# benjjneb/dada2

Hardware: AMD Instinct MI355X
Metric: unique reads denoised/sec (dada() wall-clock) (higher is better)
Workload: dtype int32 DP + f64 lambda/p-value

## Files before the change

### dada2_amd/_lib.py

```python
from __future__ import annotations

import ctypes as C
import os

from .opts import COpts

os.environ.setdefault("GPU_MAX_HW_QUEUES", "8")

_HERE = os.path.dirname(os.path.abspath(__file__))
LIB_PATH = os.path.join(_HERE, "libdada2hip.so")
_lib = None


class Dada2HipError(RuntimeError):
    def __init__(self, code, msg):
        super().__init__(msg)
        self.code = code


class CStats(C.Structure):
    _fields_ = [
        ("ncompare", C.c_uint64), ("nskipped", C.c_uint64), ("nshroud", C.c_uint64), ("ngapless", C.c_uint64),
        ("nnw", C.c_uint64), ("nshuffle", C.c_uint64), ("nstored", C.c_uint64),
        ("rounds", C.c_uint32), ("kernel_times_sampled", C.c_uint32),
        ("ms_total", C.c_double), ("ms_upload", C.c_double), ("ms_screen", C.c_double), ("ms_nw", C.c_double),
        ("ms_gapless", C.c_double), ("ms_bookkeep", C.c_double), ("ms_pval", C.c_double), ("ms_final", C.c_double),
        ("nw_kernel_ms", C.c_double), ("nw_kernel_launches", C.c_uint64), ("nw_cells", C.c_uint64),
        ("screen_kernel_ms", C.c_double), ("screen_kernel_launches", C.c_uint64), ("screen_bytes", C.c_uint64),
        ("dev_ms_screen", C.c_double), ("dev_ms_nw", C.c_double), ("dev_ms_shuffle", C.c_double),
        ("dev_ms_pval", C.c_double), ("dev_ms_birth", C.c_double), ("dev_ms_final", C.c_double),
        ("ms_wait_device", C.c_double), ("ms_replay", C.c_double), ("ms_enqueue", C.c_double),
        ("nmoves", C.c_uint64), ("batch_compares", C.c_uint64),
        ("nnw_run", C.c_uint64), ("ngapless_run", C.c_uint64),
        ("lite_chains", C.c_uint64), ("lite_misses", C.c_uint64),
        ("tail_launches", C.c_uint64), ("tail_pauses", C.c_uint64), ("tail_levels", C.c_uint64),
        ("tail_blocks", C.c_uint32), ("tail_fallbacks", C.c_uint32),
        ("dev_ms_tail", C.c_double), ("tail_ms_entry", C.c_double), ("tail_ms_shuffle0", C.c_double),
        ("tail_ms_shuffle_more", C.c_double), ("tail_ms_pupdate", C.c_double), ("tail_ms_barriers", C.c_double),
        ("tail_ms_birth", C.c_double), ("tail_ms_publish", C.c_double), ("tail_ms_release", C.c_double),
        ("pf_compares", C.c_uint64), ("pf_hits", C.c_uint64), ("pf_waits", C.c_uint64), ("pf_exits", C.c_uint64),
        ("pf_centres", C.c_uint64), ("tail_threads", C.c_uint32), ("overlap_on", C.c_uint32),
        ("dev_ms_pf_screen", C.c_double), ("dev_ms_pf_nw", C.c_double),
        ("tail_xcd_barrier", C.c_uint32), ("tail_mirror", C.c_uint32),
        ("ms_setup", C.c_double), ("ms_round0", C.c_double), ("tail_ms_pf_wait", C.c_double), ("tail_ms_pf_plan", C.c_double),
        ("nnw_retry", C.c_uint64), ("nnw_fast", C.c_uint64), ("screen_stage2", C.c_uint64), ("nnw_rounds", C.c_uint64),
    ]

    def as_dict(self):
        return {k: getattr(self, k) for k, _ in self._fields_ if not k.startswith("reserved")}


EXCHANGE_FN = C.CFUNCTYPE(C.c_int, C.c_void_p, C.c_int32, C.c_void_p, C.c_int64, C.c_void_p)


LOG_FN = C.CFUNCTYPE(None, C.c_char_p, C.c_void_p)
ABORT_FN = C.CFUNCTYPE(C.c_int, C.c_void_p)


class CHooks(C.Structure):
    _fields_ = [("log", LOG_FN), ("should_abort", ABORT_FN), ("user", C.c_void_p)]


def make_hooks(log=None, should_abort=None):
    if log is None and should_abort is None:
        return None, None
    keep = {"error": None}

    def _log(msg, _user):
        try:
            if log is not None:
                log(msg.decode(errors="replace"))
        except BaseException as ex:
            keep["error"] = keep["error"] or ex

    def _abort(_user):
        try:
            return 1 if (should_abort is not None and should_abort()) else 0
        except BaseException as ex:
            keep["error"] = keep["error"] or ex
            return 1

    h = CHooks(LOG_FN(_log), ABORT_FN(_abort), None)
    keep["cb"] = (h.log, h.should_abort)
    return h, keep


class CShard(C.Structure):
    _fields_ = [("rank", C.c_int32), ("world", C.c_int32), ("exchange", EXCHANGE_FN), ("user", C.c_void_p)]


EXPORTS = [
    "dada2hip_dada_uniques", "dada2hip_sample_create", "dada2hip_sample_set_priors", "dada2hip_sample_run",
    "dada2hip_sample_free", "dada2hip_sample_run_sharded", "dada2hip_sample_nraw", "dada2hip_sample_maxlen", "dada2hip_result_nclust",
    "dada2hip_result_nraw", "dada2hip_result_maxlen", "dada2hip_result_ncol", "dada2hip_result_nbirth_subs",
    "dada2hip_result_sequence", "dada2hip_result_abundance", "dada2hip_result_n0", "dada2hip_result_n1",
    "dada2hip_result_nunq", "dada2hip_result_clust_pval", "dada2hip_result_birth_from", "dada2hip_result_birth_pval",
    "dada2hip_result_birth_fold", "dada2hip_result_birth_ham", "dada2hip_result_birth_qave", "dada2hip_result_center",
    "dada2hip_result_bs_pos", "dada2hip_result_bs_ref", "dada2hip_result_bs_sub", "dada2hip_result_bs_qual",
    "dada2hip_result_bs_clust", "dada2hip_result_subqual", "dada2hip_result_clusterquals", "dada2hip_result_map",
    "dada2hip_result_pval", "dada2hip_result_stats", "dada2hip_result_free", "dada2hip_nwalign", "dada2hip_nwvec",
    "dada2hip_sample_compare", "dada2hip_launch_ledger", "dada2hip_nw_ring_trips", "dada2hip_sample_final_worklist", "dada2hip_calc_pA", "dada2hip_version", "dada2hip_run_multi", "dada2hip_trim_cache",
    "dada2hip_table_bimera2", "dada2hip_is_bimera", "dada2hip_bimera_pairs", "dada2hip_derep_fastq", "dada2hip_derep_nuniques",
    "dada2hip_derep_nreads", "dada2hip_derep_maxlen", "dada2hip_derep_seqs", "dada2hip_derep_abundances",
    "dada2hip_derep_quals", "dada2hip_derep_map", "dada2hip_derep_free", "dada2hip_sample_from_derep",
    "dada2hip_merge_pairs", "dada2hip_mergers_nrow", "dada2hip_mergers_sequence", "dada2hip_mergers_abundance",
    "dada2hip_mergers_forward", "dada2hip_mergers_reverse", "dada2hip_mergers_nmatch", "dada2hip_mergers_nmismatch",
    "dada2hip_mergers_nindel", "dada2hip_mergers_prefer", "dada2hip_mergers_accept", "dada2hip_mergers_free",
    "dada2hip_collapse_nomismatch", "dada2hip_collapse_pairs", "dada2hip_nweval",
    "dada2hip_taxonomy_train", "dada2hip_taxonomy_free", "dada2hip_taxonomy_table", "dada2hip_taxonomy_assign",
    "dada2hip_species_open", "dada2hip_species_free", "dada2hip_species_match", "dada2hip_species_hits_offsets",
    "dada2hip_species_hits_refs", "dada2hip_species_hits_free",
    "dada2hip_filter_open", "dada2hip_filter_free", "dada2hip_filter_reads", "dada2hip_filter_fastq", "dada2hip_filter_fastq_paired",
    "dada2hip_filter_reads_oriented", "dada2hip_filter_fastq_oriented", "dada2hip_filter_fastq_paired_ex",
    "dada2hip_primers_reads", "dada2hip_primers_fastq",
    "dada2hip_derep_combine", "dada2hip_sample_set_prior_seqs", "dada2hip_sample_prior_seqs_stats",
    "dada2hip_qprofile_reads", "dada2hip_qprofile_fastq", "dada2hip_qprofile_ncycle", "dada2hip_qprofile_counts",
    "dada2hip_qprofile_reads_total", "dada2hip_qprofile_profiled", "dada2hip_qprofile_qual_offset", "dada2hip_qprofile_free",
    "dada2hip_complexity_reads", "dada2hip_complexity_fastq", "dada2hip_complexity_free",
    "dada2hip_bimera_denovo", "dada2hip_bimera_worklist_probe", "dada2hip_bimera_fold_probe",
    "dada2hip_derep_reads", "dada2hip_filter_derep_fastq", "dada2hip_filter_derep_fastq_paired",
    "dada2hip_seqtab_merge", "dada2hip_seqtab_nrow", "dada2hip_seqtab_ncol", "dada2hip_seqtab_cells", "dada2hip_seqtab_sequences",
    "dada2hip_seqtab_samples", "dada2hip_seqtab_free",
    "dada2hip_merge_run", "dada2hip_merge_run_nsamples", "dada2hip_merge_run_nrow", "dada2hip_merge_run_column", "dada2hip_merge_run_sequences",
    "dada2hip_merge_run_free",
]

BIMERA_DENOVO_NSTATS = 16
BIMERA_DENOVO_STATS = ("sequences", "rows", "queries", "pairs_possible", "pairs_aligned", "windows", "launches", "flagged", "aligner_route",
                       "per", "slot_budget", "pack_us", "device_us", "kernel_device_us", "total_us")

PRIOR_SEQS_NSTATS = 16
PRIOR_SEQS_STATS = ("given", "kept", "keys", "keys_in_lds", "flags_set", "blocks", "pack_us", "device_us", "kernel_device_us", "total_us")


class CDerepView(C.Structure):
    _fields_ = [("nuniques", C.c_int32), ("maxlen", C.c_int32), ("nreads", C.c_int64), ("seqs", C.c_void_p),
                ("abundances", C.c_void_p), ("quals", C.c_void_p), ("map", C.c_void_p)]

COLLAPSE_NSTATS = 16
COLLAPSE_STATS = ("columns_dedup", "candidate_pairs", "pairs_scanned", "pairs_screened_out", "pairs_bound_rejected", "pairs_aligned",
                  "aligned_ham0", "batches", "join_us", "scan_us", "align_us", "resolve_us", "total_us")

TAXONOMY_NSTATS = 16
TAXONOMY_TRAIN_STATS = ("build_us", "upload_us", "table_bytes")
TAXONOMY_STATS = ("classified", "slab_queries", "gather_queries", "took_reverse_complement", "launches", "prepare_us", "slab_device_us",
                  "gather_device_us", "try_rc_device_us", "total_us")

SPECIES_NSTATS = 16
SPECIES_STATS = ("references", "bases", "windows", "windows_past_bitmap", "candidates", "candidate_reruns", "hits", "launches",
                 "seed_host_us", "seed_device_us", "verify_host_us", "verify_device_us", "total_us", "resident_bytes")

FILTER_NSTATS = 32
FILTER_STAGES = ("kept", "max_len", "trim_left", "trim_right", "trunc_q", "trunc_len", "min_len", "max_n", "min_q", "max_ee", "rm_phix",
                 "rm_lowcomplex")
FILTER_STATS = ("reads_in", "reads_kept") + tuple("dropped_" + s for s in FILTER_STAGES[1:]) + (
    "table_keys", "table_in_lds", "upload_bytes", "upload_us", "scan_device_us", "ee_device_us", "kmers_device_us", "download_us",
    "parse_us", "deflate_us", "write_us", "total_us", "open_inflate_us")


class CFilterParams(C.Structure):
    _fields_ = [("trunc_q", C.c_int32), ("trunc_len", C.c_int32), ("trim_left", C.c_int32), ("trim_right", C.c_int32),
                ("max_len", C.c_int32), ("min_len", C.c_int32), ("max_n", C.c_int32), ("min_q", C.c_int32),
                ("max_ee", C.c_double), ("rm_lowcomplex", C.c_double),
                ("rm_phix", C.c_int32), ("min_matches", C.c_int32), ("non_overlapping", C.c_int32), ("kmer_size", C.c_int32),
                ("qual_offset", C.c_int32), ("reserved", C.c_int32)]


PRIMERS_NSTATS = 24
PRIMER_CODES = ("kept", "no_fwd", "no_rev", "nothing_left", "bad_letter")
PRIMERS_STATS = ("reads_in", "reads_kept") + tuple("dropped_" + s for s in PRIMER_CODES[1:]) + (
    "flipped", "multiple_matches", "hits_fwd", "hits_rev", "pieces", "tiles", "upload_bytes", "upload_us", "kernel_device_us",
    "download_us", "parse_us", "deflate_us", "write_us", "total_us", "open_inflate_us")


class CPrimerParams(C.Structure):
    _fields_ = [("primer_fwd", C.c_char_p), ("primer_rev", C.c_char_p), ("max_mismatch", C.c_int32), ("trim_fwd", C.c_int32),
                ("trim_rev", C.c_int32), ("orient", C.c_int32), ("allow_indels", C.c_int32), ("reserved", C.c_int32)]


READQC_NSTATS = 16
QPROFILE_NSCORE = 94
READQC_STATS = ("reads_in", "reads_profiled", "pieces", "cycles", "upload_bytes", "upload_us", "kernel_device_us", "download_us", "parse_us",
                "total_us", "open_inflate_us")


SEQTAB_NSTATS = 24
SEQTAB_STATS = ("tables", "input_columns", "distinct_sequences", "flagged_sequences", "output_rows", "output_columns", "table_capacity",
                "rebuilds", "collision_rounds", "rc_failed_compares", "pieces", "upload_bytes", "download_bytes", "upload_us", "identity_us",
                "rc_lookup_us", "accumulate_us", "download_us", "total_us")

MERGE_NSTATS = 16
MERGE_STATS = ("samples", "read_pairs_in", "pairs_na", "unique_pairs", "chunks", "accepted", "table_capacity", "collisions", "upload_bytes",
               "download_bytes", "upload_us", "tally_us", "align_us", "eval_us", "download_us", "total_us")

DEREP_NSTATS = 16
DEREP_STATS = ("reads_in", "uniques", "table_capacity", "rebuilds", "collision_rounds", "pieces", "upload_bytes", "download_bytes", "upload_us",
               "kernel_device_us", "download_us", "finalise_us", "total_us")


class CSampleInput(C.Structure):
    _fields_ = [("nraw", C.c_int32), ("quals_nrow", C.c_int32), ("seqs", C.POINTER(C.c_char_p)),
                ("abundances", C.c_void_p), ("priors", C.c_void_p), ("quals", C.c_void_p)]
# ... 215 lines not shown
```

### dada2_amd/csrc/driver.cpp

```cpp
#include <fcntl.h>
#include <sys/file.h>
#include <unistd.h>

#include <algorithm>
#include <atomic>
#include <chrono>
#include <condition_variable>
#include <exception>
#include <functional>
#include <mutex>
#include <cmath>
#include <cstdarg>
#include <cstdio>
#include <cstring>
#include <ctime>
#include <memory>
#include <thread>
#include <unordered_map>

#include "engine.h"
#include "hostpar.h"
#include "knobs.h"
#include "marshal.h"
#include "ppois.h"
// ... 1240 lines not shown
    const double pA = (have ? p0 : 1.0) * N;
    if (pA < o.omegaA && have) { b.yes = true; b.type = 'A'; b.c = c; b.pval = pA; }
    else {
      BudTie cp;
      double p1 = 1.0;
      const bool havep = pick(1, cp, p1);
      const double pP = havep ? p1 : 1.0;
      if (pP < o.omegaP && havep) { b.yes = true; b.type = 'P'; b.c = cp; b.pval = pP; }
    }
    if (b.yes) b.newi = nclust_dev;
    return b;
  }

  void launch_birth(const Birth &b) {
    const int raw = b.c.raw;
    if (b.newi >= ccap) grow_clusters(std::max(ccap * 2, b.newi + 1));
    const int ev = ev_begin(EV_BIRTH, profile_all);
    launch_apply_bud(P, s->D, d_creads_snap.p, raw, b.newi, b.c.from, s->h_reads[raw], b.c.from_reads - s->h_reads[raw],
                     s->d_ctab.p, ro_next()->cnt, s->stream);
    ev_end(ev);
    nclust_dev = b.newi + 1;
    snap_fresh = true;
    ri ^= 1;
    if (shard) {
      if ((int)h_upd.size() <= b.newi) h_upd.resize(b.newi + 1, 0);
      h_upd[b.newi] = 1; h_upd[b.c.from] = 1;
    }
  }

  void confirm_auto_birth(const Birth &b) {
    if (b.type != 'A' || b.c.raw != h_rout.p->bud.ties[0][0].raw || !spec_launched)
      throw RuntimeErr{DADA2HIP_ERR_RUNTIME, "dada2hip: internal error: device and host bud decisions differ"};
    nclust_dev = b.newi + 1;
    snap_fresh = true;
    ri ^= 1;
    confirm_spec(b.newi, b.c.raw);
  }

  void record_birth(const Birth &b) {
    const int raw = b.c.raw;
    const int from = clust_of[raw];
    if (from != b.c.from) throw RuntimeErr{DADA2HIP_ERR_RUNTIME, "dada2hip: internal error: host/device membership diverged"};
    const double expected = b.c.comp_lam * bi[from].reads;
    Bi &bf = bi[from];
    const int slot = slot_of[raw];
    const uint32_t last = bf.raw.back();
    bf.raw[slot] = last;
    slot_of[last] = slot;
    bf.raw.pop_back();
    bf.reads -= s->h_reads[raw];
    bi.emplace_back();
    const int newi = (int)bi.size() - 1;
    Bi &nb = bi[newi];
    nb.birth_type = b.type;
    nb.birth_from = b.type == 'A' ? (uint32_t)from : 0u;
    nb.birth_pval = b.pval; nb.birth_fold = s->h_reads[raw] / expected; nb.birth_e = expected;
    nb.birth_comp = Comp{(uint32_t)b.c.comp_i, (uint32_t)raw, b.c.comp_lam, b.c.comp_ham};
    nb.raw.push_back((uint32_t)raw);
    nb.reads = s->h_reads[raw];
    nb.center = (uint32_t)raw;
    slot_of[raw] = 0;
    clust_of[raw] = newi;
    if (slot == 0) push_slot0();
    if (b.type == 'A') logf(", Division (naive): Raw %d from Bi %d, pA=%.2e", raw, from, b.pval);
    else logf(", Division (prior): Raw %d, pP=%.2e", raw, b.pval);
  }

  void check_errflag(int32_t f) {
    if (f & 1) throw RuntimeErr{DADA2HIP_ERR_RUNTIME, "Bad lambda."};
    if (f & 2) throw RuntimeErr{DADA2HIP_ERR_RUNTIME, "dada2hip: comparison store overflow"};
    if (f & 32) throw RuntimeErr{DADA2HIP_ERR_RUNTIME, "dada2hip: internal error: a work list of a batch compare overflowed (the compare ran twice?)"};
    if (f & 16) throw RuntimeErr{DADA2HIP_ERR_RUNTIME, "dada2hip: internal error: the persistent tail's LDS mirror disagrees with the state arrays"};
  }

  bool use_v2 = false;
  Eng2 E2{}, E2L{};
  DevBuf<double> v2_lam0, v2_lam1;
  DevBuf<uint32_t> v2_ham0, v2_ham1;
  DevBuf<int32_t> v2_i1;
  DevBuf<unsigned long long> v2_smask;
  DevBuf<int32_t> v2_head, v2_blkcount, v2_dlt, v2_movers, v2_slotc, v2_sig, v2_n0d, v2_blist, v2_blistn;
  DevBuf<unsigned long long> v2_retrytot;
  DevBuf<int32_t> v2_bretry, v2_bretryn;
  DevBuf<double> v2_lamB;
  DevBuf<uint32_t> v2_hamB;
  DevBuf<uint8_t> v2_moved;
  DevBuf<uint32_t> v2_statpart;
  DevBuf<CompBlk> v2_blk;
  DevBuf<Ctl2> v2_ctl;
  DevBuf<BudTie> v2_tiesrec;
  DevBuf<Round2Out> v2_dblk;
  DevBuf<uint16_t> v2_bcls, v2_full, v2_ord;
  DevBuf<uint2> v2_tab8;
  DevBuf<uint32_t> v2_cbits, v3_pf_cbits;
  PinBuf<Round2Out> v2_hblk;
  DevBuf<unsigned long long> v2_trace;
  int v2_trace_seq = -1;
  int v2_nbuf = 64, v2_depth = 2, v2_chain = SH_CHAIN;
  bool v2_debug = false;
  bool v3_on = false;
  int v3_depth = 1;
  int v3_grid = 1;
  long v3_enq = 0;
  long v3_ord_seen = 0;
  DevBuf<PSync> v3_psync;
  DevBuf<int32_t> v3_lockbuf;
  int v3_lock_stride = 0;
  bool v3_overlap = false;
  Eng2 E2P{};
  SampleDev S2{};
  DevBuf<Ctl2> v3_pfctl;
  DevBuf<PfSync> v3_pfsync;
  DevBuf<uint2> v3_pf_tab8;
  DevBuf<uint16_t> v3_pf_full, v3_pf_ord, v3_pf_foff;
  DevBuf<int32_t> v3_pf_blist, v3_pf_blistn, v3_pf_bretry, v3_pf_bretryn;
  DevBuf<uint32_t> v3_pf_ad;
  DevBuf<AdDesc> v3_pf_fdesc;
  long v3_pf_launched = 0;
  long v3_pf_seen = 0;
  long v3_pf_chains = 0;
  bool v3_pf_gate_on = true;
  hipEvent_t v3_pf_ev[4] = {nullptr, nullptr, nullptr, nullptr};
  DevBuf<unsigned long long> v3_ktime;
  PinBuf<int32_t> v3_hflags;
  bool v3_slot_held = false;
  int v3_slot_blocks = 0;
  long v2_enq = 0, v2_cons = 0;
  uint64_t v2_miss_launches = 0;
  struct EnqRec { int ev_screen, ev_nw; bool compare; };
  std::vector<EnqRec> v2_enqrec;

  bool want_v2() const {
    if (knobs().engine_classic) return false;
    if (plain || no_auto || !rounds_use_coop()) return false;
    if (s->D.N < 2) return false;
    return true;
  }
  void v2_bind() {
    E2.P = P; E2.S = s->D;
    E2.T.lam0 = v2_lam0.p; E2.T.ham0 = v2_ham0.p; E2.T.lam1 = v2_lam1.p; E2.T.ham1 = v2_ham1.p; E2.T.i1 = v2_i1.p; E2.T.smask = v2_smask.p; E2.T.head = v2_head.p; E2.T.blk = v2_blk.p; E2.T.blk_count = v2_blkcount.p;
    E2.T.blk_cap = (int32_t)std::min<size_t>(v2_blk.n, 0x7FFFFFF0u);
    E2.C.NBUF = v2_nbuf; E2.C.bcls = v2_bcls.p; E2.C.slot_centre = v2_slotc.p;
    E2.C.tab8 = v2_tab8.p; E2.C.full = v2_full.p; E2.C.ord = v2_ord.p; E2.C.cbits = v2_cbits.p; E2.C.Npad = ((size_t)N + 31) & ~(size_t)15;
    E2.C.lamB = v2_lamB.p; E2.C.hamB = v2_hamB.p; E2.blist = v2_blist.p; E2.blist_n = v2_blistn.p; E2.bretry = v2_bretry.p; E2.bretry_n = v2_bretryn.p; E2.fast_ctl = v2_retrytot.p;
    E2.ctl = v2_ctl.p; E2.dblk = v2_dblk.p; E2.hblk = v2_hblk.p; E2.dlt = v2_dlt.p; E2.movers = v2_movers.p;
    E2.partial = d_partial.p; E2.ties0 = d_ties0.p; E2.ties1 = d_ties1.p; E2.ccap = ccap;
    E2.sig_list = v2_sig.p + 4; E2.sig_n = v2_sig.p; E2.ties_rec = v2_tiesrec.p;
    E2.greedy = o.greedy; E2.detect_singletons = o.detect_singletons;
    E2.total_reads = (double)(uint32_t)s->total_reads; E2.omegaA = o.omegaA; E2.omegaP = o.omegaP;
    E2.bp = BudParams{o.min_fold, o.omegaA, o.omegaP, o.min_hamming, o.min_abund};
    E2.sp = sp; E2.thresh = d_thresh_round.p; E2.max_shuffle = MAX_SHUFFLE;
    E2.trace = v2_trace.p; E2.trace_seq = v2_trace_seq;
    E2.moved = v2_moved.p; E2.n0d = v2_n0d.p; E2.stat_part = v2_statpart.p; E2.stat_n = v2_n0d.p + 2 * SH_LEVELS;
    E2.psync = v3_psync.p; E2.hcons = v3_hflags.p; E2.hexit = v3_hflags.p ? v3_hflags.p + 16 : nullptr; E2.ktime = v3_ktime.p;
    E2.sh_filter = 1; E2.grid_shuffle = 2048; E2.grid_pupdate = 1024;
    const Knobs &K = knobs();
    if (K.v2_filter >= 0) E2.sh_filter = K.v2_filter;
    if (K.v2_grid_shuffle > 0) E2.grid_shuffle = std::min(8192, K.v2_grid_shuffle);
    E2.grid_shuffle = std::max<int>(E2.grid_shuffle, (int)std::min<long long>(8192, (long long)N / (256ll * 1000) + 1));
    if (K.v2_grid_pupdate > 0) E2.grid_pupdate = K.v2_grid_pupdate;
    E2.mov_inline = MOV_INLINE2; E2.ring_limit = RING2;
    if (K.v2_mov_inline > 0) E2.mov_inline = std::min(MOV_INLINE2, K.v2_mov_inline);
    if (K.v3_ring > 0) E2.ring_limit = std::min(RING2, K.v3_ring);
    E2.fail_ordinal = K.v3_fail_entry > 0 ? K.v3_fail_entry : 0;
    E2.grid_wait_ticks = (unsigned long long)((2.0 + (double)N / 1e6) * 1e8);
    E2.spec_lock_buf = v3_lockbuf.p; E2.spec_lock_stride = v3_lock_stride;
    E2.spec_eval = K.v3_spec != 0 ? 1 : 0;
    {
      const long long per_group = 4096ll * std::max(1, v3_grid);
      const long long per_block = ((long long)N + per_group - 1) / per_group * 4096ll;
      E2.mirror_on = (v3_on && K.v3_mirror != 0 && N < (1 << 24) && per_block <= (long long)tail_mirror_cap(s->device)) ? (K.v3_mirror == 2 ? 2 : 1) : 0;
    }
    E2.xbar = K.v3_xbar >= 0 ? K.v3_xbar : (v3_grid >= 48 ? 1 : 0);
    E2.spec_max_prev = K.v3_spec_max >= 0 ? K.v3_spec_max : 16;
    E2.pf_on = v3_overlap ? 1 : 0; E2.pf_min = 2; E2.pf_plan = E2.pf_on;
    E2.pf_early = K.v3_pf_early >= 0 ? K.v3_pf_early : 4;
    E2.pf_sync = K.v3_pf_sync != 0 ? 1 : 0;
    E2.pf_ctl = v3_pfctl.p; E2.pf_blist_n = v3_pf_blistn.p; E2.pfsync = v3_pfsync.p;
    {
      const double us = K.v3_pf_wait_us >= 0 ? (double)K.v3_pf_wait_us : 100.0;
      E2.pf_wait_ticks = (unsigned long long)(us * 100.0);
      v3_pf_gate_on = K.v3_pf_gate_us != 0;
      E2.pf_gate_ticks = (unsigned long long)((K.v3_pf_gate_us > 0 ? (double)K.v3_pf_gate_us : 5000.0) * 100.0);
    }
    E2.has_compare = 1;
    E2.align_at_commit = v2_align_commit ? 1 : 0;
    E2L = E2; E2L.has_compare = 0;
    if (v3_overlap) {
      S2 = s->D; S2.ad_ptr = v3_pf_ad.p; S2.ad_foff = v3_pf_foff.p; S2.ad_desc = v3_pf_fdesc.p;
      E2P = E2; E2P.S = S2; E2P.ctl = v3_pfctl.p; E2P.C.tab8 = v3_pf_tab8.p; E2P.C.full = v3_pf_full.p; E2P.C.ord = v3_pf_ord.p; E2P.C.cbits = v3_pf_cbits.p;
      E2P.blist = v3_pf_blist.p; E2P.blist_n = v3_pf_blistn.p; E2P.bretry = v3_pf_bretry.p; E2P.bretry_n = v3_pf_bretryn.p; E2P.pf_on = 0; E2P.has_compare = 1;
    }
  }
  void v2_alloc(int max_clust) {
    const size_t n = (size_t)N;
    v2_nbuf = 64;
    {
      size_t total_b = 0;
      int dev_ = 0;
      (void)hipGetDevice(&dev_);
      if (hipDeviceTotalMem(&total_b, dev_) != hipSuccess || !total_b) { (void)hipGetLastError(); total_b = (size_t)64 << 30; }
      const size_t per_buf = (((size_t)N + 31) & ~(size_t)15) * (2 + (size_t)KB_MAX * 12);
      v2_nbuf = (int)std::max<size_t>(2, std::min<size_t>(64, total_b / 8 / std::max<size_t>(per_buf, 1)));
    }
    const Knobs &K = knobs();
    if (K.v2_nbuf > 0) v2_nbuf = std::min(64, K.v2_nbuf);
    v2_depth = K.v2_depth > 0 ? std::min(MOV_RING - 1, K.v2_depth) : 2;
    v3_depth = K.v2_depth > 0 ? v2_depth : 1;
    v2_chain = K.v2_chain > 0 ? std::min(SH_CHAIN, K.v2_chain) : SH_CHAIN;
    v2_debug = K.v2_debug;
    hipStream_t stq = s->stream;
    v2_lam0.alloc(n); v2_ham0.alloc(n); v2_lam1.alloc(n); v2_ham1.alloc(n); v2_i1.alloc(n); v2_smask.alloc(n); v2_head.alloc(n); v2_blkcount.alloc(1);
    {
      size_t cap0 = std::max<size_t>(4 * n, (size_t)1 << 16);
      if (K.node_cap > 0) cap0 = std::max<size_t>((size_t)K.node_cap, n + 16);
      if (v2_blk.n < cap0) v2_blk.alloc(cap0);
    }
    v2_ctl.alloc(1); v2_dblk.alloc(RING2); v2_hblk.alloc(RING2);
    v2_dlt.alloc((size_t)SH_LEVELS * ccap);
    v2_movers.alloc((size_t)std::max(MOV_RING * SH_CHAIN, SH_LEVELS) * 3 * n);
    const size_t slots = (size_t)v2_nbuf * KB_MAX;
    v2_bcls.alloc((size_t)v2_nbuf * (((size_t)N + 31) & ~(size_t)15));
    v2_lamB.alloc(slots * (((size_t)N + 31) & ~(size_t)15)); v2_hamB.alloc(slots * (((size_t)N + 31) & ~(size_t)15));
    v2_blist.alloc((size_t)2 * KB_MAX * (((size_t)N + 31) & ~(size_t)15)); v2_blistn.alloc(2 * KB_MAX);
    v2_bretry.alloc((size_t)KB_MAX * (((size_t)N + 31) & ~(size_t)15)); v2_bretryn.alloc(KB_MAX);
    D2_HIP(hipMemsetAsync(v2_blistn.p, 0, 2 * KB_MAX * 4, stq));
    D2_HIP(hipMemsetAsync(v2_bretryn.p, 0, KB_MAX * 4, stq));
    v2_retrytot.alloc(4);
    D2_HIP(hipMemsetAsync(v2_retrytot.p, 0, 32, stq));
    v2_slotc.alloc(slots); v2_tab8.alloc(NKMER); v2_cbits.alloc(KB_MAX * 32); v2_full.alloc((size_t)KB_MAX * NKMER); v2_ord.alloc((size_t)KB_MAX * s->D.LK + 64);
    v2_sig.alloc(n + 4); v2_tiesrec.alloc((size_t)2 * TIES_FULL);
    v2_moved.alloc(n); v2_n0d.alloc(2 * SH_LEVELS + 4); v2_statpart.alloc((size_t)4 * 8192);
    D2_HIP(hipMemsetAsync(v2_moved.p, 0, n, stq));
    D2_HIP(hipMemsetAsync(v2_n0d.p, 0, (2 * SH_LEVELS + 4) * 4, stq));
    D2_HIP(hipMemsetAsync(v2_sig.p, 0, 16, stq));
    D2_HIP(hipMemsetAsync(v2_blkcount.p, 0, 4, stq));
    D2_HIP(hipMemsetAsync(v2_dblk.p, 0, sizeof(Round2Out) * RING2, stq));
    D2_HIP(hipMemsetAsync(v2_dlt.p, 0, (size_t)SH_LEVELS * ccap * 4, stq));
    D2_HIP(hipMemsetAsync(v2_slotc.p, 0xFF, slots * 4, stq));
    for (int k = 0; k < RING2; k++) v2_hblk.p[k].seq = 0;
    Ctl2 c;
    memset(&c, 0, sizeof c);
    c.nclust = 1; c.centre = (int32_t)bi[0].center; c.slot = 0; c.max_clust = max_clust;
    c.n0 = N; c.low0 = N; c.need_compare = 0; c.nalign = 0; c.abuf = 0; c.stable = 1; c.bfrom = 0;
    c.pf_bbuf = -1; c.last_bbuf = -1; c.prev_bbuf = -1;
    for (int k = 0; k < KB_MAX; k++) c.acentre[k] = -1;
    for (int k = 0; k < KB_MAX; k++) c.bcentre[k] = -1;
    D2_HIP(hipMemcpyAsync(v2_ctl.p, &c, sizeof c, hipMemcpyHostToDevice, stq));
    D2_HIP(hipStreamSynchronize(stq));
    v2_trace_seq = -1;
    if (K.v2_trace_on) {
      v2_trace_seq = K.v2_trace_seq;
      v2_trace.alloc((size_t)TRACE_KERNELS * TRACE_BLOCKS * 8);
      D2_HIP(hipMemsetAsync(v2_trace.p, 0, (size_t)TRACE_KERNELS * TRACE_BLOCKS * 64, stq));
    }
    v2_enq = v2_cons = 0;
    v2_next_full = 0;
    v2_lite_on = true;
    if (K.v2_lite >= 0) v2_lite_on = K.v2_lite != 0;
    v2_align_commit = nw_ad_apw(s->D, ap) == 1;
    if (K.v2_align >= 0) v2_align_commit = K.v2_align == 1;
    if (v2_align_commit) v2_lite_on = false;
    v2_plain_rounds = 0;
    v2_miss_launches = 0;
    v2_enqrec.clear();
    v3_setup(stq);
    v2_bind();
  }

  void v3_setup(hipStream_t stq) {
    const Knobs &K = knobs();
    v3_on = !K.v2_tail_chain;
    if (v2_trace_seq >= 0 || K.v2_trace_on) v3_on = false;

    v3_grid = tail_grid(N, s->device);
    if (K.v3_grid > 0) v3_grid = std::min(K.v3_grid, tail_grid(1 << 30, s->device));
    v3_overlap = v3_on && !v2_align_commit && v2_nbuf >= 4 && K.v3_overlap != 0 && N >= 2 && (active_runs(s->device).load() <= 1 || K.v3_overlap == 1);
    {
      const int ncu = tail_grid(1 << 30, s->device);
      if (v3_overlap && K.v3_grid == 0 && v3_grid > ncu / 2) v3_grid = std::max(1, std::min((N + 8191) / 8192, ncu / 2));
    }
    if (v3_on) { const int cap = tail_resident_max(s->device); if (cap == 0 || (cap > 0 && v3_grid > cap)) v3_on = false; }
    if (!v3_on) v3_overlap = false;
    v3_lock_stride = 0;
    if (v3_on) {
      const long long per_group = 4096ll * v3_grid;
      v3_lock_stride = (int)(((long long)N + per_group - 1) / per_group * 4096ll);
      v3_lockbuf.alloc((size_t)v3_lock_stride * (size_t)v3_grid);
    }
    v3_pf_launched = 0; v3_pf_seen = 0; v3_pf_chains = 0;
    if (v3_overlap) {
      if (!s->cmp) D2_HIP(hipStreamCreateWithFlags(&s->cmp, hipStreamNonBlocking));
      for (auto &e : v3_pf_ev) if (!e) D2_HIP(hipEventCreateWithFlags(&e, hipEventDisableTiming));
      const size_t npad = ((size_t)N + 31) & ~(size_t)15;
      v3_pfctl.alloc(1); v3_pfsync.alloc(1); v3_pf_tab8.alloc(NKMER); v3_pf_cbits.alloc(KB_MAX * 32); v3_pf_full.alloc((size_t)KB_MAX * NKMER);
      v3_pf_ord.alloc((size_t)KB_MAX * s->D.LK + 64); v3_pf_blist.alloc((size_t)2 * KB_MAX * npad); v3_pf_blistn.alloc(2 * KB_MAX);
      v3_pf_bretry.alloc((size_t)KB_MAX * npad); v3_pf_bretryn.alloc(KB_MAX);
      D2_HIP(hipMemsetAsync(v3_pf_bretryn.p, 0, KB_MAX * 4, stq));
      v3_pf_ad.alloc((size_t)s->D.ad_waves * s->D.ad_wpw);
      v3_pf_foff.alloc((size_t)s->D.ad_fcap * s->D.ad_fstride); v3_pf_fdesc.alloc((size_t)s->D.ad_fcap);
      D2_HIP(hipMemsetAsync(v3_pf_fdesc.p, 0xFF, (size_t)s->D.ad_fcap * sizeof(AdDesc), stq));
      D2_HIP(hipMemsetAsync(v3_pfctl.p, 0, sizeof(Ctl2), stq));
      D2_HIP(hipMemsetAsync(v3_pfsync.p, 0, sizeof(PfSync), stq));
      D2_HIP(hipMemsetAsync(v3_pf_blistn.p, 0, 2 * KB_MAX * 4, stq));
    }
    v3_psync.alloc(1); v3_hflags.alloc(64); v3_ktime.alloc(KT_N);
    D2_HIP(hipMemsetAsync(v3_psync.p, 0, sizeof(PSync), stq));
    D2_HIP(hipMemsetAsync(v3_ktime.p, 0, KT_N * 8, stq));
    for (int k = 0; k < 64; k++) v3_hflags.p[k] = 0;
    v3_enq = 0; v3_ord_seen = 0;
  }
  bool v3_acquire() {
    if (v3_slot_held) return true;
    v3_slot_blocks = v3_grid;
    persistent_slot(s->device).acquire(std::max(1, knobs().v3_slots), v3_slot_blocks, tail_grid(1 << 30, s->device));
    if (!persistent_file(s->device).try_acquire(s->device)) { persistent_slot(s->device).release(v3_slot_blocks); return false; }
    v3_slot_held = true;
    return true;
  }
  void v3_release() {
    if (v3_slot_held) { persistent_file(s->device).release(); persistent_slot(s->device).release(v3_slot_blocks); v3_slot_held = false; }
  }
  void v3_quiesce() {
    if (!v2_ctl.p || !s) return;
    v3_hflags.p[24] = 1;
    *(volatile int32_t *)(v3_hflags.p + 32) = 1;
    (void)hipMemcpyAsync(&v2_ctl.p->state, v3_hflags.p + 24, 4, hipMemcpyHostToDevice, s->side);
    (void)hipStreamSynchronize(s->side);
    (void)hipStreamSynchronize(s->stream);
    if (s->cmp) (void)hipStreamSynchronize(s->cmp);
    (void)hipGetLastError();
    v3_pf_release();
  }
  void v3_pf_release() {
    v3_pf_ad.free(); v3_pf_foff.free(); v3_pf_fdesc.free(); v3_pf_blist.free(); v3_pf_bretry.free();
  }
  void v3_fallback() {
    sync_spin(s->stream);
    if (v3_overlap) {
      *(volatile int32_t *)(v3_hflags.p + 32) = 1;
      sync_spin(s->cmp);
      v3_pf_totals();
      v3_overlap = false;
      v2_bind();
      v3_pf_release();
    }
    D2_HIP(hipMemsetAsync(v3_psync.p, 0, sizeof(PSync), s->stream));
    launch2_resume(E2, s->stream, true, true);
    v3_release();
    v3_on = false;
    st.tail_fallbacks++;
    v2_enq = v2_cons;
    v2_enqrec.assign((size_t)v2_cons, EnqRec{-1, -1, false});
    v2_next_full = 0;
    if (knobs().v2_summary) fprintf(stderr, "[v3] entry barrier failed after %ld blocks: continuing on the launch chains\n", v2_cons);
  }
  bool v3_block_ready() const { return *(volatile int32_t *)&v2_hblk.p[v2_cons % RING2].seq == (int32_t)(v2_cons + 1); }
  long v3_ended() const { return (long)*(volatile int32_t *)(v3_hflags.p + 16); }
  std::vector<EnqRec> v3_rec;
  void v3_enqueue(bool first) {
    const auto t_enq = clk::now();
    hipStream_t stq = s->stream;
    EnqRec rec{-1, -1, !first};
    if (!first) {
      rec.ev_screen = ev_begin(EV_SCREEN, profile_all, true);
      launch2_screen_multi(E2, stq);
      ev_end(rec.ev_screen);
      launch2_batch_lists(E2, stq);
      const NwBatch nb{&v2_ctl.p->nalign, v2_blistn.p, v2_blist.p, v2_ctl.p->acentre, &v2_ctl.p->abuf, E2.C.Npad, v2_bretry.p, v2_bretryn.p, v2_retrytot.p, &v2_ctl.p->fast_off};
      launch_gapless_batch(s->D, nb, ap, s->d_err.p, v2_lamB.p, v2_hamB.p, &v2_ctl.p->state, stq);
      rec.ev_nw = ev_begin(EV_NW, profile_all, true);
      launch_nw_ad(s->D, -1, nullptr, nullptr, nullptr, 0, nullptr, nullptr, ap, s->d_err.p, v2_lamB.p, v2_hamB.p, nullptr, 0, 0, nullptr, stq,
                   &v2_ctl.p->state, &nb);
      ev_end(rec.ev_nw);
    }
    const int ev = ev_begin(EV_TAIL, profile_all);
    Eng2 Ek = E2;
    if (!profile_all) Ek.ktime = nullptr;
    Ek.pf_plan = (v3_overlap && (active_runs(s->device).load() <= 1 || knobs().v3_overlap == 1)) ? 1 : 0;
    launch3_tail(Ek, v3_grid, first, (int)(v3_enq + 1), s->h_reads[bi[0].center], stq);
    ev_end(ev);
    v3_rec.push_back(rec);
    v3_enq++;
    st.ms_enqueue += ms_since(t_enq);
  }

  void v3_pf_enqueue(long k) {
    const auto t_enq = clk::now();
    hipStream_t st2 = s->cmp;
    Ctl2 *pc = v3_pfctl.p;
    *(volatile int32_t *)(v3_hflags.p + 40 + (k & 7)) = 0;
    launch2_pf_gate(E2P, (int)k, v3_hflags.p + 32, v3_hflags.p + 40 + (k & 7), st2);
    launch2_pf_tables(E2P, st2);
    int ev = ev_begin(EV_PF_SCREEN, profile_all, false, false, st2);
    launch2_screen_multi(E2P, st2);
    ev_end(ev);
    launch2_batch_lists(E2P, st2);
    const NwBatch nb{&pc->nalign, v3_pf_blistn.p, v3_pf_blist.p, pc->acentre, &pc->abuf, E2.C.Npad, v3_pf_bretry.p, v3_pf_bretryn.p, v2_retrytot.p, &pc->fast_off};
    launch_gapless_batch(S2, nb, ap, s->d_err.p, v2_lamB.p, v2_hamB.p, &pc->state, st2);
    ev = ev_begin(EV_PF_NW, profile_all, false, false, st2);
    launch_nw_ad(S2, -1, nullptr, nullptr, nullptr, 0, nullptr, nullptr, ap, s->d_err.p, v2_lamB.p, v2_hamB.p, nullptr, 0, 0, nullptr, st2,
                 &pc->state, &nb);
    ev_end(ev);
    launch2_pf_done(E2P, st2);
    D2_HIP(hipEventRecord(v3_pf_ev[k & 3], st2));
    v3_pf_launched = std::max(v3_pf_launched, k);
    v3_pf_chains++;
    st.ms_enqueue += ms_since(t_enq);
  }
  int v3_pf_gate_result(long k) const { return (int)*(volatile int32_t *)(v3_hflags.p + 40 + (k & 7)); }
  int32_t v3_pf_stat[4] = {0, 0, 0, 0};
  void v3_pf_totals() {
    PfSync ps;
    D2_HIP(hipMemcpy(&ps, v3_pfsync.p, sizeof ps, hipMemcpyDeviceToHost));
    st.nnw_run += ps.nnw; st.ngapless_run += ps.ngapless;
    st.pf_compares = (uint64_t)v3_pf_seen;
    st.pf_hits = (uint64_t)v3_pf_stat[0]; st.pf_waits = (uint64_t)v3_pf_stat[1]; st.pf_exits = (uint64_t)v3_pf_stat[2]; st.pf_centres = (uint64_t)v3_pf_stat[3];
    st.overlap_on = 1;
  }
  void v3_pf_serve(const Round2Out &b) {
    if (!v3_overlap) return;
    for (int k = 0; k < 4; k++) v3_pf_stat[k] = b.pf_stat[k];
    v3_pf_seen = std::max(v3_pf_seen, (long)b.pf_seq);
    if (v3_pf_seen >= 1) {
      if (v3_pf_launched < v3_pf_seen) v3_pf_enqueue(v3_pf_seen);
      else if (v3_pf_gate_result(v3_pf_seen) == 2) v3_pf_enqueue(v3_pf_seen);
    }
    if (v3_pf_gate_on && (active_runs(s->device).load() <= 1 || knobs().v3_overlap == 1) && v3_pf_launched == v3_pf_seen &&
        (v3_pf_seen == 0 || v3_pf_gate_result(v3_pf_seen) == 1))
      v3_pf_enqueue(v3_pf_seen + 1);
    if (b.pf_wait > 0 && (long)b.pf_wait <= v3_pf_launched) D2_HIP(hipStreamWaitEvent(s->stream, v3_pf_ev[b.pf_wait & 3], 0));
  }

  bool v3_dev_halted = false;

  void v3_topup() {
    if (v3_dev_halted) return;
    const long need = (long)v3_depth - (v3_enq - v3_ended());
    for (long k = 0; k < need; k++) v3_enqueue(false);
  }
  const Round2Out &v3_wait_block() {
    const int ring = (int)(v2_cons % RING2);
    const int32_t want = (int32_t)(v2_cons + 1);
    volatile int32_t *seqp = &v2_hblk.p[ring].seq;
    const auto tw = clk::now();
    const bool polite = wait_blocks();
    int burst = 0;
    for (unsigned spins = 0; *seqp != want; spins++) {
      if (v3_enq - v3_ended() < v3_depth && burst < 256) { v3_enqueue(false); burst++; continue; }
      cpu_relax();
      if (polite && spins > 64) { struct timespec ts{0, 20000}; nanosleep(&ts, nullptr); }
      if ((spins & 0xFFFF) == 0xFFFF || (polite && (spins & 0xFF) == 0xFF)) {
        hipError_t e = hipStreamQuery(s->stream);
        if (e != hipSuccess && e != hipErrorNotReady)
          throw d2::DeviceError{DADA2HIP_ERR_DEVICE, std::string("HIP error: ") + hipGetErrorString(e) + " (round result)"};
        if (e == hipSuccess && *seqp != want) {
          if (v3_ended() < v3_enq || burst >= 2) {
            PSync ps;
            D2_HIP(hipMemcpy(&ps, v3_psync.p, sizeof ps, hipMemcpyDeviceToHost));
            if (ps.fail == 1u) throw TailEntryFailed{};
            if (ps.fail != 0u || v3_ended() < v3_enq || burst >= 512)
              throw d2::DeviceError{DADA2HIP_ERR_DEVICE, "dada2hip: the persistent round tail ended without publishing its result (a grid barrier timed out?)"};
          }
          v3_enqueue(false); burst++; continue;
        }
        if (ms_since(tw) > wait_timeout_s() * 1e3)
          throw d2::DeviceError{DADA2HIP_ERR_DEVICE, "dada2hip: timed out waiting for the round result"};
      }
    }
    std::atomic_thread_fence(std::memory_order_acquire);
    v2_cons++;
    st.ms_wait_device += ms_since(tw);
    return v2_hblk.p[ring];
  }

  void run_v3(int max_clust) {
    struct SlotGuard { Run *r; ~SlotGuard() { if (r->v3_running) r->v3_quiesce(); r->v3_release(); r->v3_running = false; } } slot_guard{this};
    v3_running = true;
    auto t0 = clk::now();
    st.nstored = (uint64_t)N;
    v3_rec.clear();
    if (v3_overlap && v3_pf_gate_on && (active_runs(s->device).load() <= 1 || knobs().v3_overlap == 1)) v3_pf_enqueue(1);
    v3_enqueue(true);
    bool done = false;
    long n_halt[8] = {0, 0, 0, 0, 0, 0, 0, 0}, n_pause = 0, n_blocks = 0;
    while (!done) {
      for (int burst = 0; !v3_dev_halted && v3_enq - v3_ended() < v3_depth && burst < 4; burst++) v3_enqueue(false);
      const long seq = v2_cons + 1;
      const Round2Out *bp = nullptr;
      try { bp = &v3_wait_block(); }
      catch (const TailEntryFailed &) {
        v3_running = false;
        v3_fallback();
        st.ms_bookkeep += ms_since(t0);
        run_v2(max_clust, true, v2_cons == 0);
        return;
      }
      const Round2Out &b = *bp;
      n_blocks++;
      v3_pf_serve(b);
      if (hooks && hooks->should_abort && hooks->should_abort(hooks->user))
        throw RuntimeErr{DADA2HIP_ERR_ABORTED, "dada2hip: aborted by caller"};
      if (v2_debug)
        fprintf(stderr, "[v3] blk %ld launch %d halt %d paused %d nclust %d nsh %d cnt %d %d %d %d nbatch %d slot %d birth %d found %d nties %d p %.3e blk %d\n", seq,
                b.kord, b.halt, b.paused, b.nclust, b.nsh, b.cnt[0], b.cnt[1], b.cnt[2], b.cnt[3], b.nbatch, b.slot, b.birth_applied, b.bud.found[0],
                b.bud.nties[0], b.bud.best_p[0], b.blk_count);
      v3_dev_halted = b.halt != H2_NONE;
      v2_replay(b, seq, b.paused != 0 && b.halt == H2_NONE);
      n_halt[b.halt & 7]++;
      if (b.kord > v3_ord_seen) {
        v3_ord_seen = b.kord;
        const EnqRec &rec = v3_rec[(size_t)b.kord - 1];
        if (rec.compare && b.pad0[1] + b.pad0[2] > 0) {
          if (rec.ev_nw >= 0) evs[rec.ev_nw].ok = 1;
          st.nnw_run += (uint64_t)b.pad0[1]; st.ngapless_run += (uint64_t)b.pad0[2];
        }
        if (rec.compare && b.nbatch > 0) {
          v2_miss_launches++;
          if (rec.ev_screen >= 0) evs[rec.ev_screen].ok = 1;
        }
      }
      switch (b.halt) {
        case H2_NONE: {
          Birth bb = decide_bud(b.bud);
          if (!bb.yes || bb.type != 'A' || bb.c.raw != b.bud.ties[0][0].raw)
            throw RuntimeErr{DADA2HIP_ERR_RUNTIME, "dada2hip: internal error: device and host bud decisions differ"};
          logf("\nNew Cluster C%i:", bb.newi);
          nclust_dev = bb.newi + 1;
          record_birth(bb);
          st.ncompare += (uint64_t)N;
          if (b.paused) n_pause++;
          break;
        }
        case H2_NO_BIRTH: {
          Birth bb = decide_bud(b.bud);
          if (bb.yes) throw RuntimeErr{DADA2HIP_ERR_RUNTIME, "dada2hip: internal error: device and host bud decisions differ"};
          done = true;
          break;
        }
        case H2_MAXCLUST: done = true; break;
        case H2_HOST_DECIDE:
        case H2_CAPACITY: {
          if (b.halt == H2_CAPACITY) v2_grow(b);
          Birth bb = decide_bud(b.bud);
          if (!bb.yes) { done = true; break; }
          if (bb.newi + 2 > ccap) v2_grow(b);
          logf("\nNew Cluster C%i:", bb.newi);
          launch2_host_birth(E2, bb.c.raw, bb.c.from, s->stream);
          nclust_dev = bb.newi + 1;
          record_birth(bb);
          st.ncompare += (uint64_t)N;
          break;
        }
        case H2_FAIL: throw d2::DeviceError{DADA2HIP_ERR_DEVICE, "dada2hip: a grid barrier of the persistent round tail timed out (blocks not co-resident?)"};
        default: throw RuntimeErr{DADA2HIP_ERR_RUNTIME, "dada2hip: internal error: unexpected halt code from the persistent round tail"};
      }
      v3_dev_halted = false;
      *(volatile int32_t *)v3_hflags.p = (int32_t)v2_cons;
    }
    v3_running = false;
    sync_spin(s->stream);
    if (v3_overlap) {
      *(volatile int32_t *)(v3_hflags.p + 32) = 1;
      sync_spin(s->cmp);
      v3_pf_totals();
      v3_pf_release();
    }
    if (profile_all && v3_ktime.p) {
      unsigned long long kt[KT_N];
      D2_HIP(hipMemcpy(kt, v3_ktime.p, sizeof kt, hipMemcpyDeviceToHost));
      const double ms = 1e3 / 1e8;
      st.tail_ms_shuffle0 = kt[KT_S0] * ms; st.tail_ms_shuffle_more = kt[KT_SL] * ms; st.tail_ms_pupdate = kt[KT_P] * ms;
      st.tail_ms_barriers = (kt[KT_S0_BAR] + kt[KT_SL_BAR] + kt[KT_P_BAR]) * ms; st.tail_ms_birth = kt[KT_BIRTH] * ms;
      st.tail_ms_publish = kt[KT_PUBLISH] * ms; st.tail_ms_entry = kt[KT_LAUNCH] * ms;
      st.tail_levels = kt[KT_LEVELS]; st.tail_ms_release = kt[KT_RELEASE] * ms;
      st.tail_ms_pf_wait = kt[KT_PFWAIT] * ms; st.tail_ms_pf_plan = kt[KT_PLAN] * ms;
      if (knobs().v2_summary) {
        fprintf(stderr, "[v3] block-0 sub-phase ms (kid: 1 commit+shuffle0, 2 later shuffles, 5 p-update, 6 serial end):");
        for (int kid : {1, 2, 5, 6}) { fprintf(stderr, "  kid%d:", kid); for (int ph = 1; ph < 8; ph++) fprintf(stderr, " %.2f", kt[KT_SUB + 8 * kid + ph] * ms); }
        fprintf(stderr, "\n");
      }
    }
    st.tail_xcd_barrier = (E2.xbar && v3_grid > 1) ? 1u : 0u;
    st.tail_mirror = (v3_enq > 0 && E2.mirror_on) ? 1u : 0u;
    st.tail_launches = (uint64_t)v3_enq; st.tail_pauses = (uint64_t)n_pause; st.tail_blocks = (uint32_t)v3_grid; st.tail_threads = 1024;
    if (knobs().v2_summary && v3_overlap)
      fprintf(stderr, "[v3] overlap: prefetch compares %ld in %ld chains (centres %d)  rounds served from a prefetched batch %d  waits inside the launch %d  launches left for one %d\n",
              v3_pf_seen, v3_pf_chains, v3_pf_stat[3], v3_pf_stat[0], v3_pf_stat[1], v3_pf_stat[2]);
    if (knobs().v2_summary)
      fprintf(stderr, "[v3] blocks %ld  launches %ld  grid %d  halts none/nobirth/host/more/cap/max %ld %ld %ld %ld %ld %ld  pauses %ld  ms: wait %.1f replay %.1f enqueue %.1f total %.1f  moves %llu misses %llu\n",
              n_blocks, v3_enq, v3_grid, n_halt[0], n_halt[1], n_halt[2], n_halt[3], n_halt[4], n_halt[5], n_pause, st.ms_wait_device, st.ms_replay,
              st.ms_enqueue, ms_since(t0), (unsigned long long)st.nmoves, (unsigned long long)v2_miss_launches);
    st.ms_bookkeep += ms_since(t0);
  }

  int v2_plain_rounds = 0;
  long v2_next_full = 0;
  bool v2_lite_on = true;
  bool v2_align_commit = false;
  void v2_enqueue_chain(int nlev, bool with_compare, bool store) {
    const auto t_enq = clk::now();
    EnqRec rec{-1, -1, with_compare};
    const bool lite = with_compare && v2_lite_on && v2_plain_rounds >= 1 && v2_enq + 1 < v2_next_full;
    v2_round_launches(nlev, with_compare, store, &rec, lite);
    if (with_compare) v2_plain_rounds++;
    if (lite) st.lite_chains++;
    v2_enqrec.push_back(rec);
    v2_enq++;
    st.ms_enqueue += ms_since(t_enq);
  }
  void v2_round_launches(int nlev, bool with_compare, bool store, EnqRec *recp, bool lite = false) {
    hipStream_t stq = s->stream;
    EnqRec rec{-1, -1, with_compare};
    const Eng2 &E2 = lite ? this->E2L : this->E2;
    if (with_compare && !lite) {
      rec.ev_screen = ev_begin(EV_SCREEN, profile_all, true);
      launch2_screen_multi(E2, stq);
      ev_end(rec.ev_screen);
      launch2_batch_lists(E2, stq);
      const NwBatch nb{&v2_ctl.p->nalign, v2_blistn.p, v2_blist.p, v2_ctl.p->acentre, &v2_ctl.p->abuf, E2.C.Npad, v2_bretry.p, v2_bretryn.p, v2_retrytot.p, &v2_ctl.p->fast_off};
      launch_gapless_batch(s->D, nb, ap, s->d_err.p, v2_lamB.p, v2_hamB.p, &v2_ctl.p->state, stq);
      rec.ev_nw = ev_begin(EV_NW, profile_all, true);
      launch_nw_ad(s->D, -1, nullptr, nullptr, nullptr, 0, nullptr, nullptr, ap, s->d_err.p, v2_lamB.p, v2_hamB.p, nullptr, 0, 0, nullptr, stq,
                   &v2_ctl.p->state, &nb);
      ev_end(rec.ev_nw);
    }
    int ev = ev_begin(EV_SHUFFLE, profile_all && nlev > 0);
    for (int l = 0; l < nlev; l++) launch2_shuffle(E2, l, store && l == 0, stq);
    ev_end(ev);
    ev = ev_begin(EV_PVAL, profile_all);
    launch2_eval(E2, nlev, s->h_reads[bi[0].center], stq);
    ev_end(ev);
    if (recp) *recp = rec;
  }

  const Round2Out &v2_wait_block() {
    const int ring = (int)(v2_cons % RING2);
    const int32_t want = (int32_t)(v2_cons + 1);
    volatile int32_t *seqp = &v2_hblk.p[ring].seq;
    const auto tw = clk::now();
    const bool polite = wait_blocks();
    for (unsigned spins = 0; *seqp != want; spins++) {
      cpu_relax();
      if (polite && spins > 64) { struct timespec ts{0, 20000}; nanosleep(&ts, nullptr); }
      if ((spins & 0xFFFF) == 0xFFFF || (polite && (spins & 0xFF) == 0xFF)) {
        hipError_t e = hipStreamQuery(s->stream);
        if (e != hipSuccess && e != hipErrorNotReady)
          throw d2::DeviceError{DADA2HIP_ERR_DEVICE, std::string("HIP error: ") + hipGetErrorString(e) + " (round result)"};
        if (e == hipSuccess && *seqp != want)
          throw d2::DeviceError{DADA2HIP_ERR_DEVICE, "dada2hip: the device did not publish the round result"};
        if (ms_since(tw) > wait_timeout_s() * 1e3)
          throw d2::DeviceError{DADA2HIP_ERR_DEVICE, "dada2hip: timed out waiting for the round result"};
      }
    }
    std::atomic_thread_fence(std::memory_order_acquire);
    v2_cons++;
    st.ms_wait_device += ms_since(tw);
    return v2_hblk.p[ring];
  }

  void v2_replay(const Round2Out &b, long seq, bool resume_after_fetch = false) {
    const auto t_rep = clk::now();
    int tot = 0;
    for (int l = 0; l < b.nsh; l++) tot += b.cnt[l];
    st.nmoves += (uint64_t)tot;
    if (tot <= E2.mov_inline) {
      int off = 0;
      for (int l = 0; l < b.nsh; l++) { replay_moves(b.mov + 3 * off, b.cnt[l]); off += b.cnt[l]; }
    } else {
      const int ring = (int)((seq - 1) % MOV_RING);
      h_big.alloc((size_t)3 * tot);
      size_t off = 0;
      for (int l = 0; l < b.nsh; l++) {
        const int nm = b.cnt[l];
        if (!nm) continue;
        const size_t slot = b.kord ? (size_t)l : (size_t)(ring * SH_CHAIN + l);
        D2_HIP(hipMemcpyAsync(h_big.p + 3 * off, v2_movers.p + slot * 3 * N, (size_t)3 * nm * 4, hipMemcpyDeviceToHost, s->side));
        off += (size_t)nm;
      }
      D2_HIP(hipStreamSynchronize(s->side));
      if (resume_after_fetch) {
        launch2_resume(E2, s->stream, true);
        v3_enqueue(false);
      }
      off = 0;
      for (int l = 0; l < b.nsh; l++) { replay_moves(h_big.p + 3 * off, b.cnt[l]); off += (size_t)b.cnt[l]; }
    }
    st.nshuffle += (uint64_t)b.nsh;
    st.nnw += b.stat[0]; st.ngapless += b.stat[1]; st.nshroud += b.stat[2]; st.nskipped += b.stat[3];
    st.nnw_rounds += b.stat[0] - (uint64_t)b.pad0[3];
    st.nstored += (uint64_t)b.pad0[0];
    st.ms_replay += ms_since(t_rep);
    if (b.err_flag & 4) throw RuntimeErr{DADA2HIP_ERR_RUNTIME, "N-W Align out of range."};
    if (b.err_flag & 8) throw RuntimeErr{DADA2HIP_ERR_RUNTIME, "dada2hip: internal error: a cached compare lacks a comparison its round needs"};
    check_errflag(b.err_flag);
  }

  void v2_grow(const Round2Out &b) {
    sync_spin(s->stream);
    if (nclust_dev + 2 > ccap) {
      grow_clusters(std::max(ccap * 2, nclust_dev + 2));
      v2_dlt.alloc((size_t)SH_LEVELS * ccap);
      D2_HIP(hipMemsetAsync(v2_dlt.p, 0, (size_t)SH_LEVELS * ccap * 4, s->stream));
    }
    if ((size_t)b.blk_count + (size_t)N > v2_blk.n) {
      const size_t cap = std::max(v2_blk.n * 2, (size_t)b.blk_count + 2 * (size_t)N);
      DevBuf<CompBlk> nb;
      nb.alloc(cap);
      D2_HIP(hipMemcpyAsync(nb.p, v2_blk.p, (size_t)b.blk_count * sizeof(CompBlk), hipMemcpyDeviceToDevice, s->stream));
      D2_HIP(hipStreamSynchronize(s->stream));
      std::swap(v2_blk.p, nb.p); std::swap(v2_blk.n, nb.n);
    }
    v2_bind();
  }

  void run_v2(int max_clust, bool resume = false, bool first = true) {
    auto t0 = clk::now();
    if (!resume) st.nstored = (uint64_t)N;
    if (first) v2_enqueue_chain(0, false, false);
    bool done = false;
    double t_decide = 0, t_halt = 0, t_top = 0;
    long n_halt[8] = {0, 0, 0, 0, 0, 0, 0, 0}, n_big = 0, n_kind[5] = {0, 0, 0, 0, 0};
    while (!done) {
      const auto t_loop = clk::now();
      while (v2_enq - v2_cons < v2_depth) v2_enqueue_chain(v2_chain, true, true);
      t_top += ms_since(t_loop);
      const long seq = v2_cons + 1;
      const Round2Out &b = v2_wait_block();
      if (hooks && hooks->should_abort && hooks->should_abort(hooks->user))
        throw RuntimeErr{DADA2HIP_ERR_ABORTED, "dada2hip: aborted by caller"};
      if (b.halt == H2_NONE) while (v2_enq - v2_cons < v2_depth) v2_enqueue_chain(v2_chain, true, true);
      if (v2_debug)
        fprintf(stderr, "[v2] blk %ld halt %d nclust %d nlev %d nsh %d cnt %d %d %d %d nbatch %d slot %d birth %d found %d nties %d p %.3e blk %d\n", seq,
                b.halt, b.nclust, b.nlev, b.nsh, b.cnt[0], b.cnt[1], b.cnt[2], b.cnt[3], b.nbatch, b.slot, b.birth_applied, b.bud.found[0],
                b.bud.nties[0], b.bud.best_p[0], b.blk_count);
      if (b.halt == H2_HOST_DECIDE && knobs().v2_summary) {
        const int nt = b.bud.nties[0];
        bool zero = b.bud.found[0] && nt > 1 && nt <= BUD_TIES, in0 = false, pristine = true;
        int cmin = INT32_MAX, ncmin = 0;
        for (int k = 0; zero && k < nt; k++) {
          const BudTie &t = b.bud.ties[0][k];
          if (t.p != 0.0) zero = false;
          if (clust_of[t.raw] == 0) { in0 = true; if (slot_of[t.raw] != t.raw) pristine = false; }
          if (clust_of[t.raw] < cmin) { cmin = clust_of[t.raw]; ncmin = 1; } else if (clust_of[t.raw] == cmin) ncmin++;
        }
        n_kind[!zero ? 0 : (in0 ? (pristine ? 1 : 2) : (ncmin == 1 ? 3 : 4))]++;
      }
      v2_replay(b, seq);
      n_halt[b.halt & 7]++;
      if (b.cnt[0] + b.cnt[1] + b.cnt[2] + b.cnt[3] > MOV_INLINE2) n_big++;
      const auto t_dec = clk::now();
      const EnqRec &rec = v2_enqrec[seq - 1];
      if (rec.compare && b.pad0[1] + b.pad0[2] > 0) {
        if (rec.ev_nw >= 0) evs[rec.ev_nw].ok = 1;
        st.nnw_run += (uint64_t)b.pad0[1]; st.ngapless_run += (uint64_t)b.pad0[2];
      }
      if (rec.compare && b.nbatch > 0) {
        v2_miss_launches++;
        if (rec.ev_screen >= 0) evs[rec.ev_screen].ok = 1;
        v2_next_full = seq + b.nbatch;
      }
      if (b.nlev > 0 && b.halt != H2_SHUFFLE_MORE) { }
      switch (b.halt) {
        case H2_NONE: {
          Birth bb = decide_bud(b.bud);
          if (!bb.yes || bb.type != 'A' || bb.c.raw != b.bud.ties[0][0].raw)
            throw RuntimeErr{DADA2HIP_ERR_RUNTIME, "dada2hip: internal error: device and host bud decisions differ"};
          logf("\nNew Cluster C%i:", bb.newi);
          nclust_dev = bb.newi + 1;
          record_birth(bb);
          st.ncompare += (uint64_t)N;
          break;
        }
        case H2_NO_BIRTH: {
          Birth bb = decide_bud(b.bud);
          if (bb.yes) throw RuntimeErr{DADA2HIP_ERR_RUNTIME, "dada2hip: internal error: device and host bud decisions differ"};
          done = true;
          break;
        }
        case H2_MAXCLUST: done = true; break;
        case H2_HOST_DECIDE:
        case H2_CAPACITY: {
          v2_enq = v2_cons;
          v2_enqrec.resize((size_t)v2_cons);
          if (b.halt == H2_CAPACITY) v2_grow(b);
          Birth bb = decide_bud(b.bud);
          if (!bb.yes) { done = true; break; }
          if (bb.newi + 2 > ccap) v2_grow(b);
          logf("\nNew Cluster C%i:", bb.newi);
          launch2_host_birth(E2, bb.c.raw, bb.c.from, s->stream);
          v2_next_full = 0;
          nclust_dev = bb.newi + 1;
          record_birth(bb);
          st.ncompare += (uint64_t)N;
          break;
        }
        case H2_NEED_COMPARE: {
          v2_enq = v2_cons;
          v2_enqrec.resize((size_t)v2_cons);
          v2_next_full = 0;
          st.lite_misses++;
          launch2_resume(E2, s->stream, true);
          break;
        }
        case H2_SHUFFLE_MORE: {
          v2_enq = v2_cons;
          v2_enqrec.resize((size_t)v2_cons);
          launch2_resume(E2, s->stream);
          v2_enqueue_chain(v2_chain, false, false);
          break;
        }
        default: throw RuntimeErr{DADA2HIP_ERR_RUNTIME, "dada2hip: internal error: unknown halt code"};
      }
      if (b.halt == H2_NONE) t_decide += ms_since(t_dec); else t_halt += ms_since(t_dec);
    }
    if (knobs().v2_summary)
      fprintf(stderr, "[v2] blocks %ld  halts none/nobirth/host/more/cap/max/need-compare %ld %ld %ld %ld %ld %ld %ld  chains without compare %llu  big-mover blocks %ld  ms: wait %.1f replay %.1f "
                      "enqueue %.1f decide %.1f halt-handling %.1f top-up %.1f total %.1f  moves %llu misses %llu  host decisions other/zero-ties in partition 0 at "
                      "their first slots/... moved/elsewhere, one in the lowest partition/... several %ld %ld %ld %ld %ld\n", v2_cons, n_halt[0], n_halt[1],
              n_halt[2], n_halt[3], n_halt[4], n_halt[5], n_halt[6], (unsigned long long)st.lite_chains, n_big, st.ms_wait_device, st.ms_replay, st.ms_enqueue, t_decide, t_halt, t_top,
              ms_since(t0), (unsigned long long)st.nmoves, (unsigned long long)v2_miss_launches, n_kind[0], n_kind[1], n_kind[2], n_kind[3], n_kind[4]);
    sync_spin(s->stream);
    if (v2_trace_seq >= 0 && v2_trace.p) {
      std::vector<unsigned long long> h((size_t)TRACE_KERNELS * TRACE_BLOCKS * 8);
      D2_HIP(hipMemcpy(h.data(), v2_trace.p, h.size() * 8, hipMemcpyDeviceToHost));
      if (FILE *f = fopen(knobs().v2_trace_file.c_str(), "wb")) { fwrite(h.data(), 8, h.size(), f); fclose(f); }
    }
    st.ms_bookkeep += ms_since(t0);
  }

  uint64_t nw_cells_per_alignment() const {
    const int L = s->D.maxlen;
    if (o.band_size < 0) return (uint64_t)(L + 1) * (L + 1);
    return (uint64_t)(2 * L + 1) * (uint64_t)(o.band_size + 1);
  }
};
// ... 1229 lines not shown
```

### dada2_amd/csrc/engine.h

```cpp
#pragma once
#include <cstddef>
#include <cstdint>
#include <string>
#include <vector>

#include <hip/hip_runtime.h>

#include "../../include/dada2hip.h"
#include "merge_plain.h"

namespace d2 {

constexpr int KMER_SIZE = 5;
constexpr int NKMER = 1024;
constexpr int RANK_SAT = 63;
constexpr int MAX_SHUFFLE = 10;
constexpr int SEQLEN = 9999;
constexpr double TAIL_APPROX_CUTOFF = 1e-7;

enum : uint8_t { CLS_SKIP = 0, CLS_SHROUD = 1, CLS_GAPLESS = 2, CLS_NW = 3 };

struct DeviceError {
  int code;
  std::string msg;
// ... 88 lines not shown
                           int32_t *d_size, int32_t *d_off, int32_t *d_work, int nwork, int32_t *d_chunk_centre, hipStream_t st);
void launch_store(const PartState &P, const SampleDev &S, int ci, int centre, double total_reads, const double *d_lam,
                  const uint32_t *d_ham, const int32_t *d_round_counters, const uint8_t *d_cls, int32_t *d_zero2, hipStream_t st);
struct StoreRound {
  int ci, centre;
  double total_reads;
  const double *lam;
  const uint32_t *ham;
  const int32_t *round_counters;
  const uint8_t *cls;
};
void launch_shuffle(const PartState &P, const SampleDev &S, const uint32_t *d_creads_snap, int32_t *d_movers,
                    int32_t *d_nmovers, int32_t *d_inline, const StoreRound *store, int check_only, int nclust, hipStream_t st);
constexpr int BUD_TIES = 64;
constexpr int TIES_FULL = 4096;
struct BudTie { int32_t raw, comp_i; uint32_t comp_ham; int32_t from; uint32_t from_reads, pad; double comp_lam; double p; };
constexpr double BUD_NEAR = 1e-9;
struct BudOut {
  double best_p[2];
  uint32_t best_reads[2];
  int32_t found[2], nties[2];
  int32_t err_flag, node_count;
  int32_t valid;
  int32_t auto_applied;
  BudTie ties[2][BUD_TIES];
};
constexpr int MOVERS_INLINE = 512;
struct RoundOut {
  int32_t cnt[2];
  int32_t seq;
  int32_t pad;
  BudOut bud;
  int32_t mov[2][3 * MOVERS_INLINE];
  int32_t pad_tail[2];
};
void launch_pupdate_bud(const PartState &P, const SampleDev &S, int greedy, int detect_singletons, const BudParams &bp,
                        double init_p, uint32_t init_reads, void *d_partial, BudOut *d_out, int32_t *d_over0, int32_t *d_over1,
                        int nclust, uint8_t *d_lock_tmp, int32_t *d_check_cnt, hipStream_t st);
void launch_apply_bud(const PartState &P, const SampleDev &S, uint32_t *d_creads_snap, int raw, int newi, int from,
                      uint32_t reads_new, uint32_t reads_from, uint32_t *d_ctab, int32_t *d_zero2, hipStream_t st);
void launch_auto_birth(const PartState &P, const SampleDev &S, uint32_t *d_creads_snap, RoundOut *d_block, double omegaA, int newi,
                       uint32_t *d_ctab, int32_t *d_zero2, int32_t *d_next, RoundOut *h_block, int seq, hipStream_t st);
void launch_centre_table(const SampleDev &S, int centre, uint32_t *d_ctab, hipStream_t st);
void launch_final_p(const PartState &P, const SampleDev &S, double omegaC, uint8_t *d_correct, hipStream_t st);
void launch_posthoc(const PartState &P, const SampleDev &S, const int32_t *d_cluster_of_centre, int32_t *d_out_ji, double *d_out_lam,
                    int32_t *d_nout, int cap, hipStream_t st);

void launch_build_kmers(const SampleDev &S, hipStream_t st);
void launch_build_kmers_rows(const SampleDev &S, int r0, int r1, hipStream_t st);
void launch_screen(const SampleDev &S, int centre, const ScreenParams &sp, const uint8_t *d_skip, const uint8_t *d_lock,
                   int greedy, const int32_t *d_thresh, uint8_t *d_cls, double *d_lambda, uint32_t *d_ham, int32_t *d_nw_list,
                   int32_t *d_gl_list, int32_t *d_counters, uint32_t *d_ctab, bool build_table, const int32_t *d_centre_dev,
                   hipStream_t st);
void launch_gapless(const SampleDev &S, int centre, const int32_t *d_chunk_centre, const int32_t *d_work,
                    const int32_t *d_nwork, int nwork_host, const AlignParams &ap, const double *d_err,
                    double *d_lambda, uint32_t *d_ham, uint16_t *d_view, int LV, int view_by_chunk, hipStream_t st);

enum {
  LEDGER_AD = 0,
  LEDGER_AD_LR = 32,
  LEDGER_ADW = 64,
  LEDGER_NW = 72,
  LEDGER_NW_GEN = 88,
  LEDGER_GAPLESS = 96,
  LEDGER_WORDS = 2
};
void ledger_note(int bit);
void ledger_read(uint64_t *out, bool clear);
void nw_trips_note(int trips);
int nw_trips_read(bool clear);
void launch_pair_class(const SampleDev &S, const int32_t *d_pc, const int32_t *d_pr, int n, const ScreenParams &sp,
                       uint8_t *d_out, hipStream_t st);

struct NwScratch {
  uint32_t *ptr = nullptr;
  uint32_t *tcode = nullptr;
  int32_t *rows = nullptr;
  size_t ptr_words_per_wave = 0, t_words_per_wave = 0, row_words_per_wave = 0;
  int nwaves = 0;
};
int nw_class(int band, int maxlen, int minlen);
size_t nw_ptr_words_per_wave(int wclass, int band, int maxlen, int minlen);
void launch_nw(const SampleDev &S, int wclass, int centre, const int32_t *d_chunk_centre, const int32_t *d_work,
               const int32_t *d_nwork, int nwork_host, const AlignParams &ap, const double *d_err, const NwScratch &scr,
               double *d_lambda, uint32_t *d_ham, uint16_t *d_view, int LV, int view_by_chunk, uint8_t *d_moves,
               int moves_stride, int32_t *d_nmoves, hipStream_t st, const int32_t *d_pair_centre = nullptr);

struct NwBatch {
  const int32_t *on;
  const int32_t *n;
  const int32_t *list;
  const int32_t *centre;
  const int32_t *bbuf;
  size_t stride;
  int32_t *retry_list = nullptr;
  int32_t *retry_n = nullptr;
  unsigned long long *fast_ctl = nullptr;
  const int32_t *fast_off = nullptr;
};
void launch_gapless_batch(const SampleDev &S, const NwBatch &b, const AlignParams &ap, const double *d_err, double *d_lambda,
                          uint32_t *d_ham, const int32_t *d_stop_dev, hipStream_t st);
void launch_nw_ad(const SampleDev &S, int centre, const int32_t *d_chunk_centre, const int32_t *d_work,
                  const int32_t *d_nwork, int nwork_host, const int32_t *d_gl_work, const int32_t *d_gl_nwork,
                  const AlignParams &ap, const double *d_err, double *d_lambda, uint32_t *d_ham, uint16_t *d_view, int LV,
                  int view_by_chunk, const int32_t *d_centre_dev, hipStream_t st, const int32_t *d_stop_dev = nullptr,
                  const NwBatch *batch = nullptr);
int nw_ad_apw(const SampleDev &S, const AlignParams &ap);
size_t nw_ad_lds_bytes(const SampleDev &S, const AlignParams &ap);
void launch_nw_ad_lr(const SampleDev &S, const int32_t *d_chunk_centre, const int32_t *d_work, int nwork, const AlignParams &ap,
                     const double *d_err, int allow_one_off, int max_shift, int32_t *d_out, hipStream_t st);
size_t nw_ad_lr_lds_bytes(const SampleDev &S, const AlignParams &ap);

bool nw_adw_ok(const SampleDev &S, const AlignParams &ap);
size_t nw_adw_ptr_words_per_wave(const SampleDev &S, const AlignParams &ap);
int nw_adw_waves(const SampleDev &S, const AlignParams &ap, int nwork);
size_t nw_adw_lds_bytes(const SampleDev &S, const AlignParams &ap);
void launch_nw_adw(const SampleDev &S, int centre, const int32_t *d_chunk_centre, const int32_t *d_work, const int32_t *d_nwork,
                   int nwork_host, const AlignParams &ap, const double *d_err, uint32_t *d_ptr_scr, size_t ptr_wpw,
                   int scr_waves, double *d_lambda, uint32_t *d_ham, uint16_t *d_view, int LV, int view_by_chunk,
                   hipStream_t st);
int nw_adw_apw(const SampleDev &S, const AlignParams &ap);

constexpr int KB_MAX = 8;
constexpr int SH_CHAIN = 4;
constexpr int SH_LEVELS = MAX_SHUFFLE;
#ifndef D2_RING2
#define D2_RING2 16
#endif
constexpr int RING2 = D2_RING2;
constexpr int MOV_RING = 4;
constexpr int TRACE_BLOCKS = 4096, TRACE_KERNELS = 8;
constexpr int MOV_INLINE2 = 32768;

struct alignas(64) CompBlk {
  int32_t next, cnt;
  int32_t i[3];
  uint32_t ham[3];
  double lam[3];
  int32_t pad[2];
};
static_assert(sizeof(CompBlk) == 64, "CompBlk is one 64-byte line");
struct Store2 {
  double *lam0 = nullptr, *lam1 = nullptr;
  uint32_t *ham0 = nullptr, *ham1 = nullptr;
  int32_t *i1 = nullptr;
  unsigned long long *smask = nullptr;
  int32_t *head = nullptr;
  CompBlk *blk = nullptr;
  int32_t *blk_count = nullptr;
  int32_t blk_cap = 0;
};

enum : int32_t { H2_NONE = 0, H2_NO_BIRTH, H2_HOST_DECIDE, H2_SHUFFLE_MORE, H2_CAPACITY, H2_MAXCLUST, H2_NEED_COMPARE, H2_FAIL };

struct Ctl2 {
  int32_t state;
  int32_t halt;
  int32_t nclust;
  int32_t centre;
  int32_t slot;
  int32_t nbatch;
  int32_t bbuf;
  int32_t next_bbuf;
  int32_t pub_seq;
  int32_t nsh_base;
  int32_t max_clust;
  int32_t nalign_ran;
  int32_t nalign, abuf;
  int32_t acentre[KB_MAX];
  int32_t need_compare;
  int32_t n0, low0;
  int32_t bcentre[KB_MAX];
  uint32_t breads[KB_MAX];
  int32_t blen[KB_MAX];
  int32_t kexit, hcons_seen;
  int32_t stable, bfrom;
  int32_t pf_seq, pf_bbuf, last_bbuf, pf_wait;
  int32_t prev_bbuf;
  int32_t pf_hits, pf_spins, pf_exits, pf_centres;
  unsigned long long pf_mask;
  int32_t fast_off, fast_off_pad;
};

struct Cache2 {
  int32_t NBUF = 0;
  uint16_t *bcls = nullptr;
  int32_t *slot_centre = nullptr;
  uint2 *tab8 = nullptr;
  uint16_t *full = nullptr;
  uint16_t *ord = nullptr;
  uint32_t *cbits = nullptr;
  double *lamB = nullptr;
  uint32_t *hamB = nullptr;
  size_t Npad = 0;
};

struct Round2Out {
  int32_t seq;
  int32_t halt;
  int32_t nclust;
  int32_t birth_applied;
  int32_t nlev;
  int32_t nsh;
  int32_t cnt[SH_LEVELS];
  int32_t nbatch;
  int32_t slot;
  int32_t err_flag, blk_count;
  int32_t pad0[4];
  int32_t pf_seq;
  int32_t pf_wait;
  int32_t pf_stat[4];
  int32_t pad1[2];
  int32_t kord;
  int32_t paused;
  unsigned long long stat[4];
  BudOut bud;
  int32_t mov[3 * MOV_INLINE2];
};
static_assert(sizeof(Round2Out) % 16 == 0, "Round2Out is published as uint4s");

struct Eng2 {
  PartState P;
  SampleDev S;
  Store2 T;
  Cache2 C;
  Ctl2 *ctl;
  Round2Out *dblk;
  Round2Out *hblk;
  int32_t *dlt;
  uint8_t *moved;
  int32_t *n0d;
  int32_t *movers;
  uint32_t *stat_part;
  int32_t *stat_n;
  int32_t *blist, *blist_n;
  int32_t *bretry, *bretry_n;
  unsigned long long *fast_ctl;
  void *partial;
  int32_t *ties0, *ties1;
  BudTie *ties_rec;
  int32_t *sig_list, *sig_n;
  int32_t ccap;
  int32_t greedy, detect_singletons;
  double total_reads, omegaA, omegaP;
  BudParams bp;
  ScreenParams sp;
  const int32_t *thresh;
  int32_t max_shuffle;
  unsigned long long *trace;
  int32_t trace_seq;
  int32_t has_compare;
  int32_t align_at_commit;
  int32_t sh_filter;
  int32_t grid_shuffle, grid_pupdate;
  int32_t mov_inline;
  int32_t ring_limit;
  struct PSync *psync;
  volatile int32_t *hcons;
  volatile int32_t *hexit;
  unsigned long long *ktime;
  int32_t xbar;
  int32_t spec_max_prev;
  int32_t spec_eval;
  int32_t fail_ordinal;
  unsigned long long grid_wait_ticks;
  int32_t *spec_lock_buf;
  int32_t spec_lock_stride;
  int32_t mirror_on;
  int32_t pf_on;
  int32_t pf_plan;
  int32_t pf_min;
  int32_t pf_sync;
  int32_t pf_early;
  Ctl2 *pf_ctl;
  int32_t *pf_blist_n;
  struct PfSync *pfsync;
  unsigned long long pf_wait_ticks;
  unsigned long long pf_gate_ticks;
};

struct PfSync {
  uint32_t done, pad0[31];
  unsigned long long nnw, ngapless;
};

struct PSync {
  uint32_t arrive, pad0[31];
  uint32_t gen, pad1[31];
  uint32_t fail, pad2[31];
  uint32_t top, pad3[31];
  uint32_t ngrp, pad4[31];
  uint32_t xarr[8][32], xgen[8][32], xcount[8][32], xn[8][32];
};
enum { KT_S0 = 0, KT_S0_BAR, KT_SL, KT_SL_BAR, KT_P, KT_P_BAR, KT_BIRTH, KT_PUBLISH, KT_ROUNDS, KT_LEVELS, KT_LAUNCH, KT_RELEASE,
       KT_PFWAIT , KT_PLAN , KT_SUB_LAST = 14, KT_SUB = 16, KT_N = 80 };

void launch2_store0(const Eng2 &E, const double *d_lam, const uint32_t *d_ham, const uint8_t *d_cls, const int32_t *d_round_counters,
                    hipStream_t st);
void launch2_screen_multi(const Eng2 &E, hipStream_t st);
void launch2_pf_gate(const Eng2 &E, int k, const int32_t *h_quit, int32_t *h_result, hipStream_t st);
void launch2_pf_tables(const Eng2 &E, hipStream_t st);
void launch2_pf_done(const Eng2 &E, hipStream_t st);
void launch2_batch_lists(const Eng2 &E, hipStream_t st);
void launch2_shuffle(const Eng2 &E, int level, bool store, hipStream_t st);
void launch2_eval(const Eng2 &E, int nlev, uint32_t init_reads, hipStream_t st);
void launch2_host_birth(const Eng2 &E, int raw, int from, hipStream_t st);
void launch2_resume(const Eng2 &E, hipStream_t st, bool keep_list = false, bool compare_done = false);
void launch2_posthoc(const Eng2 &E, const int32_t *d_cluster_of_centre, int32_t *d_out_ji, double *d_out_lam, int32_t *d_nout,
                     int cap, hipStream_t st);
int tail_grid(int N, int device);
int tail_resident_max(int device);
int tail_mirror_cap(int device);
void launch3_tail(const Eng2 &E, int grid, bool first, int ordinal, uint32_t init_reads, hipStream_t st);

void launch_bimera_lr(const SampleDev &S, const int32_t *d_chunk_centre, const int32_t *d_work, int nwork, const uint8_t *d_moves,
                      int stride, const int32_t *d_nmoves, int allow_one_off, int max_shift, int32_t *d_out, hipStream_t st);

void launch_collapse_join(const SampleDev &S, int row0, int nrows, const unsigned long long *d_keys, const int32_t *d_groups,
                          int ngroups, int KW, uint32_t *d_bits, hipStream_t st);
void launch_collapse_scan(const SampleDev &S, const int2 *d_pairs, int npairs, int min_overlap, int match, int mismatch, int use_bound,
                          int4 *d_out, hipStream_t st);
constexpr int TAX_THREADS = 256;
struct TaxPart { float maxlogp; int32_t ntie; uint32_t hash; int32_t genus; };
struct TaxJob {
  const float *T;
  int gpad, ngenus, ntiles, nq, npass;
  const int32_t *koff;
  const uint16_t *karr;
  const long long *boff;
  const uint16_t *bpos;
  const int32_t *qid;
  uint32_t seed_lo, seed_hi;
  TaxPart *part;
  float *best;
  int32_t *ntie, *winner;
};
bool launch_tax_sums(const TaxJob &J, int slab_positions, hipStream_t st);
void launch_tax_combine(const TaxJob &J, hipStream_t st);
constexpr int SP_BITMAP_LOG2 = 18, SP_BITMAP_WORDS = 1 << (SP_BITMAP_LOG2 - 5);
struct SpCand { int32_t ref, pos, key; };
struct SpeciesRefs {
  const uint32_t *words, *nplane;
  const long long *woff;
  const int32_t *len;
};
struct SpeciesKeys {
  const unsigned long long *keys;
  const int32_t *groups;
  int ngroups, nkeys;
  const int32_t *key_pat_off, *key_pats, *pat_woff, *pat_len, *pat_query;
  const uint32_t *pat_words;
};
void launch_species_bitmap(const SpeciesKeys &K, uint32_t *d_bitmap, hipStream_t st);
void launch_species_seed(const SpeciesRefs &R, int r0, int r1, const SpeciesKeys &K, const uint32_t *d_bitmap, SpCand *d_cand,
                         unsigned long long cap, unsigned long long *d_counters, hipStream_t st);
void launch_species_verify(const SpeciesRefs &R, const SpeciesKeys &K, const SpCand *d_cand, unsigned long long ncand,
                           unsigned long long *d_hits, unsigned long long hit_cap, unsigned long long *d_counters, hipStream_t st);
constexpr int FT_THREADS = 1024;
constexpr int FT_LDS_MAX = 144 * 1024;
struct FilterTable {
  const unsigned long long *keys;
  const uint8_t *flags;
  int nkeys, word_size;
};
struct FilterArgs {
  int max_len, skip, trim_right, cut_char, trunc_end, min_len, max_n, minq_on, minq_char, ee_on, rm_phix, min_matches, non_overlapping;
  double max_ee;
};
struct FilterOut { int32_t code, off, len, nother, minq, hits_f, hits_r, pad; double ee; };
void launch_filter_scan(const FilterTable &T, const FilterArgs &A, int n, const uint8_t *d_seq, const uint8_t *d_qual,
                        const long long *d_off, FilterOut *d_out, hipStream_t st);
void launch_filter_ee(const FilterArgs &A, int n, const uint8_t *d_qual, const long long *d_off, const double *d_ee_tab,
                      FilterOut *d_out, hipStream_t st);
void launch_filter_kmers(int n, int k, const uint8_t *d_seq, const long long *d_off, const FilterOut *d_out, int32_t *d_counts,
                         hipStream_t st);
constexpr int FT_ORIENT_MAX = 256;
constexpr int FT_CODE_ORIENT = 12;
struct FilterBarcode {
  uint8_t fwd[FT_ORIENT_MAX], comp[FT_ORIENT_MAX];
  int len;
};
void launch_filter_orient(const FilterBarcode &B, int forward_only, int n, const uint8_t *d_seq, const long long *d_off,
                          FilterOut *d_out, hipStream_t st);
void launch_filter_scan_oriented(const FilterTable &T, const FilterArgs &A, int n, const uint8_t *d_seq, const uint8_t *d_qual,
                                 const long long *d_off, FilterOut *d_out, hipStream_t st);
void launch_filter_ee_oriented(const FilterArgs &A, int n, const uint8_t *d_qual, const long long *d_off, const double *d_ee_tab,
                               FilterOut *d_out, hipStream_t st);
void launch_filter_kmers_oriented(int n, int k, const uint8_t *d_seq, const long long *d_off, const FilterOut *d_out, int32_t *d_counts,
                                  hipStream_t st);
constexpr int PR_THREADS = 128;
constexpr int PR_MAXL = 128;
constexpr int PR_MAXMM = 15;
constexpr int PR_TILE_MAX = 64;
constexpr int PR_GRID = 4096;
constexpr int32_t PR_NA = INT32_MIN;
struct PrimerArgs {
  uint8_t sel[4][PR_MAXL];
  int32_t len[4];
  int32_t act[4], nact;
  int32_t mm, nbits, has_rev, orient, trim_fwd, trim_rev, tile;
};
struct PrimerOut { int32_t code, flip, first, last, hits[4]; };
void launch_primers(const PrimerArgs &A, int n, const uint8_t *d_seq, const long long *d_off, PrimerOut *d_out, int32_t *d_starts,
                    hipStream_t st);
constexpr int QP_NSCORE = 94;
constexpr int QP_TILE = 64;
constexpr int QP_THREADS = 1024;
constexpr int QP_ROW = QP_NSCORE + 1;
constexpr int QP_SLICE = 512;
constexpr int QP_GRID_X = 1024;
void launch_qprofile(int n, int ncyc_pad, const uint8_t *d_qual, const long long *d_off, unsigned long long *d_tab, int32_t *d_bad,
                     hipStream_t st);
constexpr int CW_WINDOW_MAX = 1024;
constexpr int CW_GRID = 16384;
struct ComplexityOut { double lo, last; };
void launch_complexity_win(int n, int k, int window, int by, const uint8_t *d_seq, const long long *d_off, const double *d_ylogy,
                           ComplexityOut *d_out, hipStream_t st);
struct PriorKeys {
  const unsigned long long *keys;
  const int32_t *groups;
  int ngroups, nkeys;
  const int32_t *key_row_off, *row_woff, *row_len, *row_seq;
  const uint32_t *row_words;
};
constexpr int PRIOR_LDS_KEYS_MAX = 6144;
int launch_prior_match(const SampleDev &S, const PriorKeys &K, bool lds, int grid_cap, const uint8_t *d_or_flags, int32_t *d_first_match,
                       hipStream_t st);
struct BimeraFold {
  const int32_t *live;
  int nq, r0, wr;
  const int32_t *work;
  const int32_t *rec;
  const int32_t *len, *P;
  int allow_one_off, min_one_off_par_dist;
  int32_t *maxima;
  uint8_t *flags;
  unsigned long long *aligned;
  int last;
  int32_t *next_live, *n_next;
};
void launch_bimera_worklist(const int32_t *d_live, int nq, int r0, int wr, int per, const int32_t *d_rank, const int32_t *d_P,
                            const uint8_t *d_flags, int32_t *d_chunk_centre, int32_t *d_work, hipStream_t st);
void launch_bimera_fold(const BimeraFold &F, hipStream_t st);
void launch_calc_pA(int n, const int32_t *d_reads, const double *d_E, const uint8_t *d_prior, double *d_out,
                    hipStream_t st);
constexpr int DD_EMPTY = -1;
constexpr int DD_PENDING = -2, DD_SKIP = -1;
struct DdRead { long long start, idx; int32_t len, pad; };
struct DdCounters { unsigned long long arena_used; int32_t nuniq, pending, err, minq; };
struct DdState {
  int32_t *tab;
  int cap;
  unsigned long long hmask;
  unsigned long long *u_hash, *u_count, *u_first, *sums;
  long long *u_off;
// ... 44 lines not shown
```

### dada2_amd/csrc/knobs.h

```cpp
#pragma once
#include <algorithm>
#include <atomic>
#include <cstdlib>
#include <cstring>
#include <memory>
#include <mutex>
#include <string>

namespace d2 {

enum { NWK_AUTO = 0, NWK_LANE = 1, NWK_COOP = 2, NWK_WIDE = 3 };

struct Knobs {
  bool engine_classic = false;
  int nw_kernel = 0;
  bool ad_homo = true;
  bool no_speculation = false;
  bool no_autobirth = false;
  int v2_nbuf = 0;
  int v2_depth = 0;
  int v2_chain = 0;
  int v2_lite = -1;
  int v2_align = -1;
  int v2_filter = -1;
  int v2_grid_shuffle = 0;
  int v2_grid_pupdate = 0;
  int v2_mov_inline = 0;
  bool v2_tail_chain = false;
  int v3_grid = 0;
  int v3_ring = 0;
  int v3_overlap = -1;
  int v3_pf_wait_us = -1;
  int v3_pf_early = -1;
  int v3_pf_gate_us = -1;
  int v3_xbar = -1;
  int v3_spec = 1;
  int v3_spec_max = -1;
  int v3_pf_sync = 0;
  int replay_radix_min = 4096;
  int v3_slots = 3;
  int v3_mirror = 1;
  int v3_fail_entry = 0;
  bool v2_debug = false;
  bool v2_summary = false;
  bool v2_trace_on = false;
  int v2_trace_seq = -1;
  std::string v2_trace_file;
  bool profile = false;
  long long node_cap = 0;
  bool wait_block = false;
  double wait_timeout_s = 600.0;
  long long ad_fcap = 0;
  int screen_bits = 1;
  int ad_fast = 1;
  long long nw_ring = 0;
  long long upload_chunk_rows = 0;
  int ad_debug = 0;
  bool bimera_times = false;
  long long bimera_slots = 0;
  int collapse_batch = 0;
  int collapse_scan = 1;
  int collapse_join = 1;
  int tax_slab = 256;
  long long tax_chunk = 0;
  long long filter_piece = 0;
  long long filter_piece_bytes = 0;
  long long primers_piece = 0;
  long long primers_piece_bytes = 0;
  long long primers_tile = 0;
  long long readqc_piece = 0;
  long long readqc_piece_bytes = 0;
  long long derep_piece = 0;
  long long derep_piece_bytes = 0;
  long long derep_table = 0;
  int derep_hash_bits = 64;
  int merge_hash_bits = 64;
  long long merge_chunk = 0;
  int species_cand = 1 << 20;
  int species_chunk = 8192;
  int priors_lds_keys = 4096;
  int priors_grid = 0;
  bool derep_zlib = false;
  bool derep_times = false;
  int host_threads = 0;
  int alloc_cache = -1;
  long long alloc_cache_gb = -1;
  std::string env_text;

  static Knobs from_env() {
    Knobs k;
    auto S = [&k](const char *n) -> const char * {
      const char *e = std::getenv(n);
      if (e) k.env_text.append(n).append(1, '=').append(e).append(1, '\n');
      return e;
    };
    auto I = [&](const char *n, int dflt) -> int { const char *e = S(n); return e ? std::atoi(e) : dflt; };
    auto B = [&](const char *n) -> bool { const char *e = S(n); return e && std::atoi(e) != 0; };
    auto T = [&](const char *n) -> int { const char *e = S(n); return e ? (std::atoi(e) != 0 ? 1 : 0) : -1; };
    if (const char *e = S("DADA2HIP_ENGINE")) k.engine_classic = !std::strcmp(e, "classic");
    if (const char *e = S("DADA2HIP_NW_KERNEL")) k.nw_kernel = !std::strcmp(e, "lane") ? 1 : (!std::strcmp(e, "coop") ? 2 : (!std::strcmp(e, "wide") ? 3 : 0));
    if (const char *e = S("DADA2HIP_AD_HOMO")) k.ad_homo = std::strcmp(e, "0") != 0;
    k.no_speculation = S("DADA2HIP_NO_SPECULATION") != nullptr;
    k.no_autobirth = S("DADA2HIP_NO_AUTOBIRTH") != nullptr;
    k.v2_nbuf = I("DADA2HIP_V2_NBUF", 0); k.v2_depth = I("DADA2HIP_V2_DEPTH", 0); k.v2_chain = I("DADA2HIP_V2_CHAIN", 0);
    k.v2_lite = T("DADA2HIP_V2_LITE");
    if (const char *e = S("DADA2HIP_V2_ALIGN")) k.v2_align = !std::strcmp(e, "commit") ? 1 : 0;
    k.v2_filter = T("DADA2HIP_V2_FILTER");
    k.v2_grid_shuffle = I("DADA2HIP_V2_GRID_SHUFFLE", 0); k.v2_grid_pupdate = I("DADA2HIP_V2_GRID_PUPDATE", 0);
    k.v2_mov_inline = I("DADA2HIP_V2_MOV_INLINE", 0);
    if (const char *e = S("DADA2HIP_V2_TAIL")) k.v2_tail_chain = !std::strcmp(e, "chain");
    k.v3_grid = I("DADA2HIP_V3_GRID", 0); k.v3_ring = I("DADA2HIP_V3_RING", 0);
    k.v3_overlap = T("DADA2HIP_V3_OVERLAP"); k.v3_pf_wait_us = I("DADA2HIP_V3_PF_WAIT_US", -1);
    k.v3_fail_entry = I("DADA2HIP_V3_FAIL_ENTRY", 0); k.v3_spec = I("DADA2HIP_V3_SPEC", 1); k.v3_xbar = T("DADA2HIP_V3_XBAR"); k.v3_spec_max = I("DADA2HIP_V3_SPEC_MAX", -1);
    k.v3_pf_early = I("DADA2HIP_V3_PF_EARLY", -1); k.v3_pf_sync = I("DADA2HIP_V3_PF_SYNC", 0); k.v3_pf_gate_us = I("DADA2HIP_V3_PF_GATE_US", -1);
    k.v3_mirror = I("DADA2HIP_V3_MIRROR", 1);
    k.v3_slots = I("DADA2HIP_V3_SLOTS", 3);
    k.replay_radix_min = I("DADA2HIP_REPLAY_RADIX_MIN", 4096);
    k.v2_debug = S("DADA2HIP_V2_DEBUG") != nullptr; k.v2_summary = S("DADA2HIP_V2_SUMMARY") != nullptr;
    if (const char *e = S("DADA2HIP_V2_TRACE")) {
      k.v2_trace_on = true; k.v2_trace_seq = std::atoi(e);
      const char *colon = std::strchr(e, ':');
      k.v2_trace_file = colon ? colon + 1 : "dada2hip_trace.bin";
    }
    k.profile = B("DADA2HIP_PROFILE");
    if (const char *e = S("DADA2HIP_NODE_CAP")) k.node_cap = std::atoll(e);
    if (const char *e = S("DADA2HIP_WAIT")) k.wait_block = !std::strcmp(e, "block");
    if (const char *e = S("DADA2HIP_WAIT_TIMEOUT_S")) k.wait_timeout_s = std::atof(e);
    if (const char *e = S("DADA2HIP_AD_FCAP")) k.ad_fcap = std::atoll(e);
    k.ad_debug = I("DADA2HIP_AD_DEBUG", 0); k.ad_fast = I("DADA2HIP_AD_FAST", 1); k.screen_bits = I("DADA2HIP_SCREEN_BITS", 1);
    if (const char *e = S("DADA2HIP_BIMERA_TIMES")) k.bimera_times = !std::strcmp(e, "1");
    k.collapse_batch = I("DADA2HIP_COLLAPSE_BATCH", 0); k.collapse_scan = I("DADA2HIP_COLLAPSE_SCAN", 1);
    k.collapse_join = I("DADA2HIP_COLLAPSE_JOIN", 1);
    k.tax_slab = I("DADA2HIP_TAX_SLAB", 256);
    auto P = [&](const char *n) -> long long { const char *e = S(n); return e ? std::max(1ll, std::atoll(e)) : 0ll; };
    k.tax_chunk = P("DADA2HIP_TAX_CHUNK"); k.filter_piece = P("DADA2HIP_FILTER_PIECE"); k.filter_piece_bytes = P("DADA2HIP_FILTER_PIECE_BYTES");
    k.upload_chunk_rows = P("DADA2HIP_UPLOAD_CHUNK_ROWS");
    k.nw_ring = P("DADA2HIP_NW_RING"); k.bimera_slots = P("DADA2HIP_BIMERA_SLOTS");
    k.primers_piece = P("DADA2HIP_PRIMERS_PIECE"); k.primers_piece_bytes = P("DADA2HIP_PRIMERS_PIECE_BYTES"); k.primers_tile = P("DADA2HIP_PRIMERS_TILE");
    k.readqc_piece = P("DADA2HIP_READQC_PIECE"); k.readqc_piece_bytes = P("DADA2HIP_READQC_PIECE_BYTES");
    k.derep_piece = P("DADA2HIP_DEREP_PIECE"); k.derep_piece_bytes = P("DADA2HIP_DEREP_PIECE_BYTES"); k.derep_table = P("DADA2HIP_DEREP_TABLE");
    k.derep_hash_bits = std::max(0, std::min(64, I("DADA2HIP_DEREP_HASH_BITS", 64)));
    k.merge_hash_bits = std::max(0, std::min(64, I("DADA2HIP_MERGE_HASH_BITS", 64))); k.merge_chunk = P("DADA2HIP_MERGE_CHUNK");
    k.species_cand = I("DADA2HIP_SPECIES_CAND", 1 << 20); k.species_chunk = I("DADA2HIP_SPECIES_CHUNK", 8192);
    k.priors_lds_keys = I("DADA2HIP_PRIORS_LDS_KEYS", 4096); k.priors_grid = I("DADA2HIP_PRIORS_GRID", 0);
    if (const char *e = S("DADA2HIP_DEREP_INFLATE")) k.derep_zlib = !std::strcmp(e, "zlib");
    if (const char *e = S("DADA2HIP_DEREP_TIMES")) k.derep_times = !std::strcmp(e, "1");
    k.host_threads = I("DADA2HIP_HOST_THREADS", 0);
    k.alloc_cache = T("DADA2HIP_ALLOC_CACHE");
    if (const char *e = S("DADA2HIP_ALLOC_CACHE_GB")) k.alloc_cache_gb = std::atoll(e);
    return k;
  }
};

namespace knobs_detail {
inline std::mutex &mu() { static std::mutex m; return m; }
inline std::atomic<const Knobs *> &cur() { static std::atomic<const Knobs *> p{nullptr}; return p; }
}

inline void knobs_process_defaults() { (void)setenv("GPU_MAX_HW_QUEUES", "8", 0); }

inline void knobs_reload() {
  Knobs k = Knobs::from_env();
  std::lock_guard<std::mutex> g(knobs_detail::mu());
  const Knobs *c = knobs_detail::cur().load(std::memory_order_relaxed);
  if (!c || c->env_text != k.env_text) knobs_detail::cur().store(new Knobs(std::move(k)), std::memory_order_release);
}
inline const Knobs &knobs() {
  const Knobs *c = knobs_detail::cur().load(std::memory_order_acquire);
  if (c) return *c;
  knobs_reload();
  return *knobs_detail::cur().load(std::memory_order_acquire);
}

}
```

### dada2_amd/csrc/rounds2.inc.hip

```cpp

#ifndef D2_PUPD_INLINE
#define D2_PUPD_INLINE __forceinline__
#endif
#ifndef D2_SHUF_INLINE
#define D2_SHUF_INLINE __forceinline__
#endif
#define D2_TRACE2(KID, SUBKID, PHASE)                                                                              \
  do {                                                                                                             \
    if (E.trace && threadIdx.x == 0 && (int)blockIdx.x < TRACE_BLOCKS && E.ctl->pub_seq == E.trace_seq)           \
      E.trace[((size_t)(KID) * TRACE_BLOCKS + blockIdx.x) * 8 + (PHASE)] = gcn_clock();                            \
    D2_KSUB(SUBKID, PHASE, blockIdx.x == 0);                                                                       \
  } while (0)
#define D2_TRACE(KID, PHASE) D2_TRACE2(KID, KID, PHASE)
#define D2_TRACE_SH(LEVEL, PHASE) D2_TRACE2(1 + (LEVEL), (LEVEL) == 0 ? 1 : 2, PHASE)
#ifdef D2_TAIL_TU
static __shared__ unsigned long long s_ktime[KT_N];
#define D2_KT s_ktime
#else
#define D2_KT E.ktime
#endif
#define D2_KSUB(KID, PHASE, WHO)                                                                                   \
  do {                                                                                                             \
    if (E.ktime && threadIdx.x == 0 && (WHO)) {                                                                    \
      const unsigned long long now_ = gcn_wall_clock();                                                            \
// ... 1169 lines not shown
      if (lost | gained) { E.n0d[2 * l] = 0; E.n0d[2 * l + 1] = 0; }
      if (n0 - lost < low0) low0 = n0 - lost;
      n0 += gained - lost;
    }
    ctl->n0 = n0; ctl->low0 = low0;
    s_hint[1] = n0; s_hint[2] = low0; s_hint[3] = 1;
  }
  D2_TRB(1);
  if (cs.eval_ok) {
    BudKey b0 = init, b1 = init;
    if (tid < nblocks) { if (bud_better(pk0.p, pk0.reads, b0)) b0 = pk0; if (bud_better(pk1.p, pk1.reads, b1)) b1 = pk1; }
    for (int k = tid + blockDim.x; k < nblocks; k += blockDim.x) {
      if (bud_better(partial[2 * k].p, partial[2 * k].reads, b0)) b0 = partial[2 * k];
      if (bud_better(partial[2 * k + 1].p, partial[2 * k + 1].reads, b1)) b1 = partial[2 * k + 1];
    }
#pragma unroll
    for (int o = 32; o >= 1; o >>= 1) {
      BudKey t;
      t.p = __shfl_xor(b0.p, o, 64); t.reads = __shfl_xor(b0.reads, o, 64);
      if (bud_better(t.p, t.reads, b0)) b0 = t;
      t.p = __shfl_xor(b1.p, o, 64); t.reads = __shfl_xor(b1.reads, o, 64);
      if (bud_better(t.p, t.reads, b1)) b1 = t;
    }
    if ((tid & 63) == 0) { s_k[0][tid >> 6] = b0; s_k[1][tid >> 6] = b1; }
    __syncthreads();
    b0 = s_k[0][0]; b1 = s_k[1][0];
    for (int k = 1; k < ((int)blockDim.x >> 6); k++) {
      if (bud_better(s_k[0][k].p, s_k[0][k].reads, b0)) b0 = s_k[0][k];
      if (bud_better(s_k[1][k].p, s_k[1][k].reads, b1)) b1 = s_k[1][k];
    }
    const bool found0 = bud_better(b0.p, b0.reads, init), found1 = bud_better(b1.p, b1.reads, init);
    const bool sig0 = b0.p * S.N < 2.0 * E.bp.omegaA, sig1 = b1.p < 2.0 * E.bp.omegaP;
    const double thr0 = sig0 ? b0.p * (1.0 + BUD_NEAR) + 2e-323 : -1.0, thr1 = sig1 ? b1.p * (1.0 + BUD_NEAR) + 2e-323 : -1.0;
    const int M = s_pre[PRE_SIGN];
    BudOut *bo = &out->bud;
    double ps_[2] = {0.0, 0.0};
    uint32_t rds_[2] = {0, 0};
    uint8_t prs_[2] = {0, 0};
#pragma unroll
    for (int j = 0; j < 2; j++) {
      const int q = tid + j * (int)blockDim.x;
      if (q >= M) sq[j] = -1;
      if (sq[j] >= 0) { ps_[j] = P.p[sq[j]]; rds_[j] = S.reads[sq[j]]; prs_[j] = S.prior[sq[j]]; }
    }
    auto consider = [&](int r, double p, uint32_t reads, bool prior) __attribute__((always_inline)) {
      for (int track = 0; track < 2; track++) {
        if (track == 1 && !prior) continue;
        const BudKey &bk = track ? b1 : b0;
        if (!(track ? (found1 && sig1) : (found0 && sig0))) continue;
        const bool exact = p == bk.p && reads == bk.reads;
        const bool near = !exact && p != 0.0 && p <= (track ? thr1 : thr0);
        if (!exact && !near) continue;
        if (near && track == 0) s_nnear = 1;
        const int k = atomicAdd(&s_nt[track], 1);
        if (k < TIES_FULL) {
          BudTie t;
          t.raw = r; t.comp_i = P.comp_i[r]; t.comp_ham = P.comp_ham[r]; t.comp_lam = P.comp_lam[r];
          t.from = P.clust_of[r]; t.from_reads = P.creads[t.from]; t.p = p; t.pad = 0;
          if (k < BUD_TIES) { bo->ties[track][k] = t; if (track == 0) s_tie[k] = t; }
          E.ties_rec[(size_t)track * TIES_FULL + k] = t;
        }
        (track ? E.ties1 : E.ties0)[k] = r;
      }
    };
#pragma unroll
    for (int j = 0; j < 2; j++) if (sq[j] >= 0) consider(sq[j], ps_[j], rds_[j], prs_[j] != 0);
    for (int q = tid + 2 * (int)blockDim.x; q < M; q += blockDim.x) {
      const int r = E.sig_list[q];
      consider(r, P.p[r], S.reads[r], S.prior[r] != 0);
    }
    __syncthreads();
    if (tid == 0) {
      bo->best_p[0] = b0.p; bo->best_p[1] = b1.p;
      bo->best_reads[0] = b0.reads; bo->best_reads[1] = b1.reads;
      bo->found[0] = found0; bo->found[1] = found1;
      bo->nties[0] = s_nt[0]; bo->nties[1] = s_nt[1];
      bo->valid = 1;
      s_k[0][0] = b0; s_k[1][0] = b1;
      s_misc[2] = found0 ? 1 : 0; s_misc[3] = found1 ? 1 : 0;
    }
  }
  __syncthreads();
  D2_TRB(2);
  if (tid == 0) {
    out->nlev = nlev; out->nsh = cs.nexec; out->slot = s_pre[PRE_SLOT]; out->nbatch = s_pre[PRE_NBATCH];
    if (s_pre[PRE_NALRAN] > 0) ctl->nalign_ran = 0;
    if ((s_pre[PRE_NALIGN] > 0 || s_pre[PRE_NALRAN] > 0) && nlev > 0) {
      int nn = 0, ng = 0;
      for (int k = 0; k < KB_MAX; k++) { nn += s_pre[PRE_BLIST + k]; ng += s_pre[PRE_BLIST + KB_MAX + k]; }
      out->pad0[1] = nn; out->pad0[2] = ng;
    }
    const int errf = s_pre[PRE_ERR] | (s_pre[PRE_NWFLAG] ? 4 : 0), blkc = s_pre[PRE_BLKCNT];
    out->err_flag = errf;
    out->blk_count = blkc;
    int halt = H2_NONE, raw = -1, from = 0;
    if (!cs.eval_ok) { halt = H2_SHUFFLE_MORE; ctl->nsh_base += cs.nexec; }
    else if (nclust >= s_pre[PRE_MAXCLUST]) halt = H2_MAXCLUST;
    else {
      const BudKey b0 = s_k[0][0], b1 = s_k[1][0];
      const bool found0 = s_misc[2] != 0, found1 = s_misc[3] != 0;
      const int nt0 = s_nt[0];
      const double pA = b0.p * S.N;
      int win = nt0 == 1 ? 0 : -1;
      if (found0 && nt0 > 1 && nt0 <= BUD_TIES && !s_nnear && b0.p == 0.0) {
        int cmin = 0x7FFFFFFF, ncmin = 0, kmin = -1, rmin = 0x7FFFFFFF;
        bool ok = true;
        const int low0 = s_hint[2];
        for (int k = 0; k < nt0; k++) {
          const int fr = s_tie[k].from, rw = s_tie[k].raw;
          if (fr < cmin) { cmin = fr; ncmin = 0; rmin = 0x7FFFFFFF; }
          if (fr == cmin) {
            ncmin++;
            if (fr == 0 && (E.moved[rw] || rw + 1 >= low0)) ok = false;
            if (rw < rmin) { rmin = rw; kmin = k; }
          }
        }
        if (ok && (ncmin == 1 || cmin == 0)) win = kmin;
      }
      if (win > 0) {
        const BudTie t = s_tie[0]; s_tie[0] = s_tie[win]; s_tie[win] = t;
        out->bud.ties[0][0] = s_tie[0]; out->bud.ties[0][win] = s_tie[win];
        win = 0;
      }
      const bool birthA = found0 && win == 0 && pA < E.omegaA * (1.0 - 1e-9);
      const bool noA = !found0 || pA >= E.omegaA * (1.0 + 1e-9);
      const bool noP = !found1 || b1.p >= E.omegaP * (1.0 + 1e-9);
      if (birthA) { raw = s_tie[0].raw; from = s_tie[0].from; s_hint[0] = (int32_t)b0.reads; }
      else if (noA && noP) halt = H2_NO_BIRTH;
      else halt = H2_HOST_DECIDE;
      if (halt == H2_NONE && (nclust + 2 > E.ccap || blkc + S.N > E.T.blk_cap)) halt = H2_CAPACITY;
    }
    if (cs.eval_ok) ctl->stable = (nlev == 0 || (cs.nexec > 0 && s_pre[PRE_CNT + cs.nexec - 1] == 0)) ? 1 : 0;
    out->halt = halt;
    out->birth_applied = halt == H2_NONE ? 1 : 0;
    out->nclust = nclust + (halt == H2_NONE ? 1 : 0);
    s_halt = halt; s_raw = raw; s_from = from; s_evalok = cs.eval_ok ? 1 : 0;
    if (halt != H2_NONE) { ctl->state = 1; ctl->halt = halt; }
  }
  __syncthreads();
  D2_TRB(3);
  if (s_evalok)
    for (int k = tid; k < nclust; k += blockDim.x) { P.update_e[k] = 0; P.check_locks[k] = 0; }
  __syncthreads();
  bool plan_due = false;
  if (s_halt == H2_NONE) plan_due = apply_birth_and_plan(E, s_raw, s_from, s_cnt, s_misc, s_hint, kord != 0);
  D2_TRB(4);
  if (kord && tid == 0) {
    int tot = 0;
    for (int l = 0; l < SH_LEVELS; l++) tot += s_pre[PRE_CNT + l];
    const bool pause = s_halt == H2_NONE && tot > E.mov_inline;
    if (pause) { out->paused = 1; ctl->state = 1; ctl->halt = H2_NONE; }
    out->kord = kord;
    const int seq = ctl->pub_seq + 1;
    int ex = (s_halt != H2_NONE || pause || ctl->need_compare != 0 || E.align_at_commit != 0 || ctl->pf_wait != 0) ? 1 : 0;
    if (!ex && seq + 1 - s_pre[PRE_HCONS] > E.ring_limit) {
      const int hc = gcn_load_system((const int32_t *)E.hcons);
      ctl->hcons_seen = hc;
      if (seq + 1 - hc > E.ring_limit) ex = 1;
    }
    ctl->kexit = ex;
  }
  clear_block(E.dblk + ((ring + 1) % RING2));
  go();
  if (plan_due) prefetch_plan_now(E, s_raw, s_misc[1] / KB_MAX, s_cnt, s_misc, true);
  __syncthreads();
  if (tid == 0) {
    if (s_halt == H2_NONE) *E.sig_n = 0;
    out->pf_seq = ctl->pf_seq; out->pf_wait = ctl->pf_wait;
    out->pf_stat[0] = ctl->pf_hits; out->pf_stat[1] = ctl->pf_spins; out->pf_stat[2] = ctl->pf_exits; out->pf_stat[3] = ctl->pf_centres;
  }
#undef D2_TRB
}

#ifndef D2_TAIL_TU
__global__ __launch_bounds__(1024) void k2_birth(Eng2 E, int nlev, BudKey init, const BudKey *__restrict__ partial, int nblocks) {
  Ctl2 *ctl = E.ctl;
  const bool halted = ctl->state != 0, starved = !E.has_compare && ctl->need_compare != 0;
  __syncthreads();
  if (halted) return;
  if (starved) {
    const int ring0 = ctl->pub_seq % RING2;
    Round2Out *o = E.dblk + ring0;
    if (threadIdx.x == 0) {
      o->halt = H2_NEED_COMPARE; o->nclust = ctl->nclust; o->birth_applied = 0; o->nlev = 0; o->nsh = 0; o->nbatch = 0; o->slot = ctl->slot;
      o->err_flag = *E.P.err_flag | (*E.S.nw_flag ? 4 : 0); o->blk_count = *E.T.blk_count;
      ctl->state = 1; ctl->halt = H2_NEED_COMPARE;
    }
    __syncthreads();
    clear_block(E.dblk + ((ring0 + 1) % RING2));
    publish_block(E, o, ring0);
    return;
  }
  if (threadIdx.x == 0) ctl->need_compare = 0;
  const int ring = ctl->pub_seq % RING2;
  Round2Out *out = E.dblk + ring;
  const Chain2 cs = chain_state(ctl, out, nlev, E.max_shuffle);
  birth_body(E, nlev, cs, init, partial, nblocks, 0);
  publish_block(E, out, ring);
}

__global__ __launch_bounds__(1024) void k2_host_birth(Eng2 E, int raw, int from) {
  __shared__ __attribute__((aligned(16))) uint32_t s_cnt[KB_MAX * NKMER];
  __shared__ int s_misc[32 + NBUF_MAX * KB_MAX];
  if (threadIdx.x == 0) { E.ctl->state = 0; E.ctl->halt = H2_NONE; }
  __syncthreads();
  apply_birth_and_plan(E, raw, from, s_cnt, s_misc);
  __syncthreads();
  if (threadIdx.x == 0) *E.sig_n = 0;
}
__global__ void k2_resume(Eng2 E, int keep_list, int compare_done) {
  E.ctl->state = 0; E.ctl->halt = H2_NONE;
  if (!keep_list) *E.sig_n = 0;
  if (compare_done) { E.ctl->nbatch = 0; E.ctl->need_compare = 0; if (!E.align_at_commit) E.ctl->nalign = 0; }
}

__global__ void k2_pf_gate(Eng2 E, int k, const int32_t *quit, int32_t *result) {
  if (threadIdx.x != 0) return;
  Ctl2 *pc = E.ctl;
  int res = 2;
  const unsigned long long t0 = gcn_wall_clock();
  for (unsigned n = 0;; n++) {
    if ((int32_t)(gcn_load_agent((const uint32_t *)&pc->pf_seq) - (uint32_t)k) >= 0) { res = 1; break; }
    if (gcn_wall_clock() - t0 > E.pf_gate_ticks || ((n & 15u) == 0u && gcn_load_system(quit) != 0)) break;
    gcn_poll_pause();
  }
  gcn_acquire_agent();
  pc->state = res == 1 ? 0 : 1;
  __hip_atomic_store(result, res, __ATOMIC_RELAXED, __HIP_MEMORY_SCOPE_SYSTEM);
}
__global__ __launch_bounds__(1024) void k2_pf_tables(Eng2 E) {
  __shared__ __attribute__((aligned(16))) uint32_t s_cnt[KB_MAX * NKMER];
  const int nb = E.ctl->nbatch;
  if (E.ctl->state != 0 || nb <= 0) return;
  build_batch_tables(E.S, E.C, nb, E.ctl->bcentre, s_cnt);
}
__global__ void k2_pf_done(Eng2 E) {
  if (threadIdx.x != 0 || E.ctl->state != 0) return;
  unsigned long long nn = 0, ng = 0;
  for (int k = 0; k < KB_MAX; k++) { nn += (unsigned long long)E.blist_n[k]; ng += (unsigned long long)E.blist_n[KB_MAX + k]; }
  E.pfsync->nnw += nn; E.pfsync->ngapless += ng;
  gcn_release_agent();
  gcn_store_agent(&E.pfsync->done, (uint32_t)E.ctl->pf_seq);
}

struct ScrIn { uint4 c0, c1; int Lr, nh; uint32_t rd; bool lk; };

template <int WAVES>
__global__ __launch_bounds__(256, WAVES) void k2_screen_multi(Eng2 E) {
  const Ctl2 *ctl = E.ctl;
  const int nb = ctl->nbatch;
  if (ctl->state != 0 || nb == 0) return;
  extern __shared__ __attribute__((aligned(16))) uint32_t s_mem[];
  const SampleDev &S = E.S;
  const Cache2 &C = E.C;
  const ScreenParams sp = E.sp;
  uint2 *tab = (uint2 *)s_mem;
  uint16_t *cord = (uint16_t *)(tab + NKMER);
  int32_t *thr = (int32_t *)(cord + (size_t)KB_MAX * S.LK);
  __shared__ int cL[KB_MAX], cC[KB_MAX];
  __shared__ uint32_t cR[KB_MAX];
  const int tid = threadIdx.x;
  for (int i = tid; i < NKMER; i += 256) tab[i] = C.tab8[i];
  {
    const int n16 = (nb * S.LK * 2 + 15) / 16;
    const uint4 *src = (const uint4 *)C.ord;
    for (int i = tid; i < n16; i += 256) ((uint4 *)cord)[i] = src[i];
  }
  for (int i = tid; i < S.maxlen + 2; i += 256) thr[i] = E.thresh[i];
  if (tid < KB_MAX) { cL[tid] = ctl->blen[tid]; cC[tid] = ctl->bcentre[tid]; cR[tid] = ctl->breads[tid]; }
  __syncthreads();
  uint16_t *bcls = C.bcls + (size_t)ctl->bbuf * C.Npad;
  const int lane = tid & 63, sub = tid & 15, g = lane >> 4;
  const int gwave = blockIdx.x * 4 + (tid >> 6), nwaves = gridDim.x * 4;
  const int nchunk = (S.maxlen - KMER_SIZE + 1 + 7) >> 3;
  const uint4 pad4 = make_uint4(0xFFFFFFFFu, 0xFFFFFFFFu, 0xFFFFFFFFu, 0xFFFFFFFFu);
  const bool heavy_on = sp.use_kmers && S.HMAX > 0;
  const int kc = sub & 7;
  const bool kvalid = sub < 8 && kc < nb;
  const int Lc = cL[kc], Cc = cC[kc];
  const uint32_t Rc = cR[kc];
  auto load = [&](int r) __attribute__((always_inline)) {
    ScrIn in;
    const bool on = r < S.N;
    const uint4 *row = (const uint4 *)(S.kord + (size_t)(on ? r : 0) * S.LK);
    in.c0 = (on && sp.use_kmers && sub < nchunk) ? row[sub] : pad4;
    in.c1 = (on && sp.use_kmers && sub + 16 < nchunk) ? row[sub + 16] : pad4;
    in.Lr = on ? S.len[r] : 0;
    in.rd = on ? S.reads[r] : 0u;
    in.lk = on && E.greedy && E.P.lock[r];
    in.nh = (on && heavy_on) ? S.nheavy[r] : 0;
    return in;
  };
  auto one = [&](int r, const ScrIn in) __attribute__((always_inline)) -> uint32_t {
    if (r >= S.N) return 0u;
    const uint4 *row = (const uint4 *)(S.kord + (size_t)r * S.LK);
    uint32_t w0 = 0, w1 = 0, w2 = 0, w3 = 0;
    if (sp.use_kmers) {
      for (int ch = sub, j = 0; ch < nchunk; ch += 16, j++) {
        const uint4 v = j == 0 ? in.c0 : (j == 1 ? in.c1 : row[ch]);
        uint32_t ax = 0, ay = 0;
        const uint32_t w[4] = {v.x, v.y, v.z, v.w};
#pragma unroll
        for (int e = 0; e < 4; e++) {
#pragma unroll
          for (int hlf = 0; hlf < 2; hlf++) {
            const uint32_t x = hlf ? (w[e] >> 16) : (w[e] & 0xFFFFu);
            const uint2 t = tab[x & 1023u];
            const uint32_t rk = x >> 10;
            const uint32_t rr = gcn_bcast_byte0(rk);
            ax += ((t.x - rr) >> 7) & 0x01010101u;
            ay += ((t.y - rr) >> 7) & 0x01010101u;
          }
        }
        w0 += ax & 0x00FF00FFu; w1 += (ax >> 8) & 0x00FF00FFu;
        w2 += ay & 0x00FF00FFu; w3 += (ay >> 8) & 0x00FF00FFu;
      }
#pragma unroll
      for (int o = 8; o >= 1; o >>= 1) {
        w0 += __shfl_xor(w0, o, 16); w1 += __shfl_xor(w1, o, 16);
        w2 += __shfl_xor(w2, o, 16); w3 += __shfl_xor(w3, o, 16);
      }
    }
    uint32_t dot = (((kc & 4) ? ((kc & 1) ? w3 : w2) : ((kc & 1) ? w1 : w0)) >> ((kc & 2) ? 16 : 0)) & 0xFFFFu;
    const bool skipped = E.greedy && (in.rd > Rc || (in.lk && r != Cc));
    if (in.nh > 0 && kvalid && !skipped) {
      for (int hh = 0; hh < in.nh; hh++) {
        const uint32_t e = S.heavy[(size_t)r * S.HMAX + hh], cr = e >> 16, cc = C.full[(size_t)kc * NKMER + (e & 1023u)];
        const uint32_t m = cr < cc ? cr : cc;
        if (m > RANK_SAT) dot += m - RANK_SAT;
      }
      dot &= 0xFFFFu;
    }
    const int d = (Lc < in.Lr ? Lc : in.Lr) - KMER_SIZE + 1;
    const bool shroud = sp.use_kmers && (int)dot < thr[d > 0 ? d : 0];
    const bool gl_ok = sp.gapless && sp.use_kmers && (sp.sse >= 1 || in.Lr == Lc);
    bool gapless = sp.band == 0;
    const bool need2 = kvalid && !skipped && !shroud && !gapless && gl_ok;
    uint32_t mask = (uint32_t)((__ballot(need2) >> (16 * g)) & 0xFFull);
    while (mask) {
      const int kk = __builtin_ctz(mask);
      mask &= mask - 1;
      const int dk = __shfl(d, kk, 16);
      const uint32_t dotk = (uint32_t)__shfl((int)dot, kk, 16);
      const uint16_t *ck = cord + (size_t)kk * S.LK;
      uint32_t ord = 0;
      for (int ch = sub, j = 0; ch < nchunk; ch += 16, j++) {
        const uint4 v = j == 0 ? in.c0 : (j == 1 ? in.c1 : row[ch]);
        const uint4 ck4 = ((const uint4 *)ck)[ch];
        const uint32_t w[4] = {v.x, v.y, v.z, v.w}, cw[4] = {ck4.x, ck4.y, ck4.z, ck4.w};
        const int i0 = ch << 3;
#pragma unroll
        for (int e = 0; e < 4; e++) {
          const uint32_t t = (w[e] ^ cw[e]) & 0x03FF03FFu;
          ord += ((t & 0xFFFFu) == 0 && i0 + 2 * e < dk);
          ord += ((t >> 16) == 0 && i0 + 2 * e + 1 < dk);
        }
      }
#pragma unroll
      for (int o = 8; o >= 1; o >>= 1) ord += __shfl_xor(ord, o, 16);
      if (kc == kk && sub < 8) gapless = (ord & 0xFFFFu) == dotk;
    }
    uint32_t c = !kvalid ? 0u : (skipped ? (uint32_t)CLS_SKIP : (shroud ? (uint32_t)CLS_SHROUD : (gapless ? (uint32_t)CLS_GAPLESS : (uint32_t)CLS_NW)));
    uint32_t code = c << (2 * kc);
    code |= __shfl_xor(code, 1, 16); code |= __shfl_xor(code, 2, 16); code |= __shfl_xor(code, 4, 16);
    return code & 0xFFFFu;
  };
  const bool pre = sp.use_kmers && S.kbits != nullptr && S.kmult != nullptr && C.cbits != nullptr;
  if (!pre) {
    for (int base16 = gwave * 16; base16 < S.N; base16 += nwaves * 16) {
      const int r0 = base16 + 4 * g;
      const ScrIn i0 = load(r0), i1 = load(r0 + 1);
      unsigned long long clsacc = one(r0, i0);
      const ScrIn i2 = load(r0 + 2);
      clsacc |= (unsigned long long)one(r0 + 1, i1) << 16;
      const ScrIn i3 = load(r0 + 3);
      clsacc |= (unsigned long long)one(r0 + 2, i2) << 32;
      clsacc |= (unsigned long long)one(r0 + 3, i3) << 48;
      if (sub == 0 && r0 < S.N) *(unsigned long long *)(bcls + r0) = clsacc;
    }
    return;
  }
  constexpr int SCR_ITERS = 8, SCR_LIST = SCR_ITERS * 64;
  __shared__ int s_list[SCR_LIST];
  __shared__ int s_nlist;
  __shared__ uint2 s_cbits[KB_MAX][16];
  if (tid < KB_MAX * 16) s_cbits[tid >> 4][tid & 15] = ((const uint2 *)C.cbits)[tid];
  if (tid == 0) s_nlist = 0;
  __syncthreads();
  const int wv = tid >> 6, grp = tid >> 4;
  auto flush = [&]() __attribute__((always_inline)) {
    __syncthreads();
    const int n = s_nlist;
    for (int q = grp; q < ((n + 15) & ~15); q += 32) {
      const bool ha = q < n, hb = q + 16 < n;
      const int ra = ha ? s_list[q] : s_list[0], rb = hb ? s_list[q + 16] : s_list[0];
      const ScrIn ia = load(ra), ib = load(rb);
      const uint32_t ca = one(ra, ia), cb = one(rb, ib);
      if (sub == 0 && ha) bcls[ra] = (uint16_t)ca;
      if (sub == 0 && hb) bcls[rb] = (uint16_t)cb;
    }
    __syncthreads();
    if (tid == 0) { if (n && E.fast_ctl) atomicAdd(&E.fast_ctl[3], (unsigned long long)n); s_nlist = 0; }
    __syncthreads();
  };
  int iter = 0;
  for (long long bb = (long long)blockIdx.x * 64; bb < S.N; bb += (long long)gridDim.x * 64, iter++) {
    const int r0 = (int)bb + 16 * wv + 4 * g;
    uint2 bw[4];
    int Ls[4], kms[4];
    uint32_t rds[4];
    bool lks[4];
#pragma unroll
    for (int u = 0; u < 4; u++) {
      const int r = r0 + u;
      const bool on = r < S.N;
      bw[u] = on ? ((const uint2 *)(S.kbits + (size_t)r * 32))[sub] : make_uint2(0u, 0u);
      Ls[u] = on ? S.len[r] : 0;
      rds[u] = on ? S.reads[r] : 0u;
      lks[u] = on && E.greedy && E.P.lock[r];
      kms[u] = on ? (int)S.kmult[r] : 0;
    }
    unsigned long long clsacc = 0;
    uint32_t survs = 0;
#pragma unroll
    for (int u = 0; u < 4; u++) {
      const int r = r0 + u;
      uint32_t p[4];
#pragma unroll
      for (int kk = 0; kk < 4; kk++) {
        const uint2 c0 = s_cbits[2 * kk][sub], c1 = s_cbits[2 * kk + 1][sub];
        const uint32_t n0 = (uint32_t)__popc(bw[u].x & c0.x) + (uint32_t)__popc(bw[u].y & c0.y);
        const uint32_t n1 = (uint32_t)__popc(bw[u].x & c1.x) + (uint32_t)__popc(bw[u].y & c1.y);
        p[kk] = n0 | (n1 << 16);
      }
#pragma unroll
      for (int o = 8; o >= 1; o >>= 1) {
        p[0] += __shfl_xor(p[0], o, 16); p[1] += __shfl_xor(p[1], o, 16);
        p[2] += __shfl_xor(p[2], o, 16); p[3] += __shfl_xor(p[3], o, 16);
      }
      const uint32_t pk = (kc & 4) ? ((kc & 2) ? p[3] : p[2]) : ((kc & 2) ? p[1] : p[0]);
      const int bound = (int)((pk >> ((kc & 1) ? 16 : 0)) & 0xFFFFu) + kms[u];
      const int d = (Lc < Ls[u] ? Lc : Ls[u]) - KMER_SIZE + 1;
      const bool skipped = E.greedy && (rds[u] > Rc || (lks[u] && r != Cc));
      const bool open = kvalid && r < S.N && !skipped && !(bound < thr[d > 0 ? d : 0]);
      uint32_t code = (kvalid ? (skipped ? (uint32_t)CLS_SKIP : (uint32_t)CLS_SHROUD) : 0u) << (2 * kc);
      code |= __shfl_xor(code, 1, 16); code |= __shfl_xor(code, 2, 16); code |= __shfl_xor(code, 4, 16);
      const bool any_open = ((__ballot(open) >> (16 * g)) & 0xFFFFull) != 0ull;
      if (any_open) survs |= 1u << u;
      clsacc |= (unsigned long long)(code & 0xFFFFu) << (16 * u);
    }
    if (sub == 0 && r0 < S.N) {
      if (survs == 0) *(unsigned long long *)(bcls + r0) = clsacc;
      else {
        int at = atomicAdd(&s_nlist, __popc(survs));
#pragma unroll
        for (int u = 0; u < 4; u++) {
          if (r0 + u >= S.N) continue;
          if ((survs >> u) & 1u) s_list[at++] = r0 + u;
          else bcls[r0 + u] = (uint16_t)(clsacc >> (16 * u));
        }
      }
    }
    if ((iter % SCR_ITERS) == SCR_ITERS - 1) flush();
  }
  flush();
}

__global__ __launch_bounds__(256) void k2_posthoc(Eng2 E, const int32_t *__restrict__ cluster_of_centre, int32_t *__restrict__ out_ji,
                                                  double *__restrict__ out_lam, int32_t *__restrict__ nout, int cap) {
  const int r = blockIdx.x * blockDim.x + threadIdx.x;
  if (r >= E.S.N) return;
  const int j = cluster_of_centre[r];
  if (j < 0) return;
  if (j != 0) {
    const int k = atomicAdd(nout, 1);
    if (k < cap) { out_ji[2 * k] = j; out_ji[2 * k + 1] = 0; out_lam[k] = E.T.lam0[r]; }
  }
  const int i1 = E.T.i1[r];
  if (i1 >= 0 && i1 != j) {
    const int k = atomicAdd(nout, 1);
    if (k < cap) { out_ji[2 * k] = j; out_ji[2 * k + 1] = i1; out_lam[k] = E.T.lam1[r]; }
  }
  for (int b = E.T.head[r], hops = 0; b >= 0 && hops < (1 << 22); b = E.T.blk[b].next, hops++) {
    const CompBlk *cb = E.T.blk + b;
    for (int q = 0; q < cb->cnt; q++) {
      const int i = cb->i[q];
      if (i == j) continue;
      const int k = atomicAdd(nout, 1);
      if (k < cap) { out_ji[2 * k] = j; out_ji[2 * k + 1] = i; out_lam[k] = cb->lam[q]; }
    }
  }
}

void launch2_store0(const Eng2 &E, const double *d_lam, const uint32_t *d_ham, const uint8_t *d_cls, const int32_t *d_round_counters,
                    hipStream_t st) {
  const int grid = std::min((E.S.N + 255) / 256, 2048);
  hipLaunchKernelGGL(k2_store0, dim3(grid), dim3(256), 0, st, E, d_lam, d_ham, d_cls, d_round_counters);
}
void launch2_batch_lists(const Eng2 &E, hipStream_t st) {
  const int grid = (E.S.N + 256 * LISTS_PER_THREAD - 1) / (256 * LISTS_PER_THREAD);
  hipLaunchKernelGGL(k2_batch_lists, dim3(grid), dim3(256), 0, st, E);
}
void launch2_pf_gate(const Eng2 &E, int k, const int32_t *h_quit, int32_t *h_result, hipStream_t st) {
  hipLaunchKernelGGL(k2_pf_gate, dim3(1), dim3(64), 0, st, E, k, h_quit, h_result);
}
void launch2_pf_tables(const Eng2 &E, hipStream_t st) { hipLaunchKernelGGL(k2_pf_tables, dim3(1), dim3(1024), 0, st, E); }
void launch2_pf_done(const Eng2 &E, hipStream_t st) { hipLaunchKernelGGL(k2_pf_done, dim3(1), dim3(64), 0, st, E); }
void launch2_screen_multi(const Eng2 &E, hipStream_t st) {
  const size_t lds = (size_t)NKMER * 8 + (size_t)KB_MAX * E.S.LK * 2 + (size_t)(E.S.maxlen + 2) * 4 + 16;
  static size_t attr_set[64] = {0};
  int dev_ = 0;
  (void)hipGetDevice(&dev_);
  if (lds > attr_set[dev_ & 63]) {
    (void)hipFuncSetAttribute((const void *)k2_screen_multi<4>, hipFuncAttributeMaxDynamicSharedMemorySize, (int)lds);
    attr_set[dev_ & 63] = lds;
  }
  const int grid = std::min((E.S.N + 63) / 64, 2048);
  hipLaunchKernelGGL(k2_screen_multi<4>, dim3(grid), dim3(256), lds, st, E);
}
void launch2_shuffle(const Eng2 &E, int level, bool store, hipStream_t st) {
  const int grid = std::min((E.S.N + 255) / 256, (int)E.grid_shuffle);
  if (store) hipLaunchKernelGGL(k2_shuffle<true>, dim3(grid), dim3(256), 0, st, E, level);
  else hipLaunchKernelGGL(k2_shuffle<false>, dim3(grid), dim3(256), 0, st, E, level);
}
void launch2_eval(const Eng2 &E, int nlev, uint32_t init_reads, hipStream_t st) {
  BudKey init{1.0, init_reads};
  const int grid = std::min((E.S.N + 255) / 256, std::min(8192, (int)E.grid_pupdate));
  hipLaunchKernelGGL(k2_pupdate, dim3(grid), dim3(256), 0, st, E, nlev, init, (BudKey *)E.partial);
  hipLaunchKernelGGL(k2_birth, dim3(1), dim3(1024), 0, st, E, nlev, init, (const BudKey *)E.partial, grid);
}
void launch2_host_birth(const Eng2 &E, int raw, int from, hipStream_t st) {
  hipLaunchKernelGGL(k2_host_birth, dim3(1), dim3(1024), 0, st, E, raw, from);
}
void launch2_resume(const Eng2 &E, hipStream_t st, bool keep_list, bool compare_done) {
  hipLaunchKernelGGL(k2_resume, dim3(1), dim3(1), 0, st, E, keep_list ? 1 : 0, compare_done ? 1 : 0);
}
void launch2_posthoc(const Eng2 &E, const int32_t *d_cluster_of_centre, int32_t *d_out_ji, double *d_out_lam, int32_t *d_nout,
                     int cap, hipStream_t st) {
  hipLaunchKernelGGL(k2_posthoc, dim3((E.S.N + 255) / 256), dim3(256), 0, st, E, d_cluster_of_centre, d_out_ji, d_out_lam, d_nout, cap);
}
#endif
```

### dada2_amd/csrc/rounds3.inc.hip

```cpp


template <int BS>
struct TailLds {
  ShufLds<BS> sh;
  PupdLds<BS> pu;
  int last, ok;
  int xtmp[8];
  int xcc, xn, ngrp;
};
struct XBar { int on; uint32_t epoch; };

enum : uint32_t { TAIL_FAIL_ENTRY = 1u, TAIL_FAIL_LATE = 2u };
static __device__ __forceinline__ void tail_fail(const Eng2 &E, uint32_t code) {
  gcn_store_agent(&E.psync->fail, code);
  E.ctl->state = 1; E.ctl->halt = H2_FAIL;
}

template <int BS, typename F>
static __device__ __forceinline__ bool grid_sync(const Eng2 &E, TailLds<BS> &L, uint32_t &epoch, int G, F &&serial, uint32_t fail_code = TAIL_FAIL_LATE,
                                                 XBar *xb = nullptr) {
  PSync *ps = E.psync;
  gcn_drain_stores();
  __syncthreads();
  const bool xmode = xb != nullptr && xb->on != 0 && G > 1;
  if (threadIdx.x == 0 && xmode) {
    int last = 0, ok = 1;
    const uint32_t e1 = xb->epoch + 1u;
    const int x = L.xcc;
    const uint32_t t = gcn_add_agent(&ps->xarr[x][0], 1u);
    if (t == e1 * (uint32_t)L.xn - 1u) {
      gcn_release_agent();
      const uint32_t t2 = gcn_add_agent(&ps->top, 1u);
      last = t2 == e1 * (uint32_t)L.ngrp - 1u;
    }
    if (!last) {
      const unsigned long long t0 = gcn_wall_clock();
      for (unsigned n = 1;; n++) {
        if ((int32_t)(gcn_load_agent(&ps->xgen[x][0]) - e1) >= 0) break;
        gcn_poll_pause();
        if ((n & 63u) == 0u && (gcn_load_agent(&ps->fail) != 0u || gcn_wall_clock() - t0 > E.grid_wait_ticks)) { ok = 0; break; }
      }
      if (!ok) tail_fail(E, fail_code);
    }
    gcn_acquire_agent();
    L.last = last; L.ok = ok;
  }
  if (threadIdx.x == 0 && !xmode) {
    int last = 1, ok = 1;
    if (G > 1) {
      const bool tm = E.ktime != nullptr && blockIdx.x == 0;
      const unsigned long long tr0 = tm ? gcn_wall_clock() : 0ull;
      gcn_release_agent();
      if (tm) s_ktime[KT_RELEASE] += gcn_wall_clock() - tr0;
      const uint32_t t = gcn_add_agent(&ps->arrive, 1u);
      last = t == (epoch + 1u) * (uint32_t)G - 1u;
      if (!last) {
        const unsigned long long t0 = gcn_wall_clock();
        for (unsigned n = 1;; n++) {
          if ((int32_t)(gcn_load_agent(&ps->gen) - (epoch + 1u)) >= 0) break;
          gcn_poll_pause();
          if ((n & 63u) == 0u && (gcn_load_agent(&ps->fail) != 0u || gcn_wall_clock() - t0 > E.grid_wait_ticks)) { ok = 0; break; }
        }
        if (!ok) tail_fail(E, fail_code);
      } else if (fail_code == TAIL_FAIL_ENTRY && gcn_load_agent(&ps->fail) != 0u) ok = 0;
      gcn_acquire_agent();
    } else {
      gcn_release_agent();
      gcn_acquire_agent();
    }
    L.last = last; L.ok = ok;
  }
  __syncthreads();
  if (!L.ok) return false;
  if (L.last) {
    bool released = false;
    auto release = [&]() __attribute__((always_inline)) {
      gcn_drain_stores();
      __syncthreads();
      if (xmode) {
        if (threadIdx.x == 0) gcn_release_agent();
        __syncthreads();
        if (threadIdx.x < 8) gcn_store_agent(&ps->xgen[threadIdx.x][0], xb->epoch + 1u);
      } else if (G > 1) {
        if (threadIdx.x == 0) { gcn_release_agent(); gcn_store_agent(&ps->gen, epoch + 1u); }
      } else {
        if (threadIdx.x == 0) { gcn_release_agent(); gcn_acquire_agent(); }
        __syncthreads();
      }
      released = true;
    };
    serial(release);
    if (!released) release();
  }
  if (xmode) xb->epoch++; else epoch++;
  return true;
}

template <int BS>
constexpr size_t tail_lds_bytes(bool mirror) { return ((sizeof(TailLds<BS>) + 15) & ~(size_t)15) + (mirror ? (size_t)MIR_CAP * 8 : 0); }

template <int BS>
static __device__ __forceinline__ void mir_fill(const Eng2 &E, uint32_t *mir) {
  constexpr int U = ShufLds<BS>::U;
  const int N = E.S.N;
  for (int grp = 0; (long long)grp * U * BS * gridDim.x < N; grp++) {
    int i1s[U], cls_[U];
    uint8_t lks[U];
    double ps_[U];
    unsigned long long sms[U];
#pragma unroll
    for (int u = 0; u < U; u++) {
      const int r = sweep_unique<BS, U>(grp, u);
      i1s[u] = -1; cls_[u] = 0; lks[u] = 0; ps_[u] = 1.0; sms[u] = 0ull;
      if (r < N) { i1s[u] = E.T.i1[r]; cls_[u] = E.P.clust_of[r]; lks[u] = E.P.lock[r]; ps_[u] = E.P.p[r]; sms[u] = E.T.smask[r]; }
    }
#pragma unroll
    for (int u = 0; u < U; u++) {
      const int slot = (grp * U + u) * BS + (int)threadIdx.x;
      mir[slot] = sweep_unique<BS, U>(grp, u) < N ? ((uint32_t)cls_[u] & MIR_CL) | (i1s[u] >= 0 ? MIR_I1 : 0u) | (lks[u] ? MIR_LOCK : 0u) | (ps_[u] != 1.0 ? MIR_PNE1 : 0u) : MIR_INVALID;
      mir[MIR_CAP + slot] = mir_fold(sms[u]);
    }
  }
  __syncthreads();
}

template <int BS>
static __device__ __forceinline__ void mir_verify(const Eng2 &E, const uint32_t *mir) {
  constexpr int U = ShufLds<BS>::U;
  const int N = E.S.N;
  __syncthreads();
  for (int grp = 0; (long long)grp * U * BS * gridDim.x < N; grp++)
    for (int u = 0; u < U; u++) {
      const int r = sweep_unique<BS, U>(grp, u);
      if (r >= N) { if (mir[(grp * U + u) * BS + (int)threadIdx.x] != MIR_INVALID) atomicOr(E.P.err_flag, 16); continue; }
      const uint32_t want = ((uint32_t)E.P.clust_of[r] & MIR_CL) | (E.T.i1[r] >= 0 ? MIR_I1 : 0u) | (E.P.lock[r] ? MIR_LOCK : 0u) | (E.P.p[r] != 1.0 ? MIR_PNE1 : 0u);
      const int slot = (grp * U + u) * BS + (int)threadIdx.x;
      if (mir[slot] != want || mir[MIR_CAP + slot] != mir_fold(E.T.smask[r])) atomicOr(E.P.err_flag, 16);
    }
}

template <int BS>
__global__ __launch_bounds__(BS, BS == 512 ? 2 : 4) void k3_tail(Eng2 E, BudKey init, int first, int ordinal) {
  extern __shared__ __attribute__((aligned(16))) unsigned char s_dyn3[];
  TailLds<BS> &L = *(TailLds<BS> *)s_dyn3;
  uint32_t *const mir = E.mirror_on ? (uint32_t *)(s_dyn3 + tail_lds_bytes<BS>(false)) : nullptr;
  gcn_raise_priority();
  Ctl2 *ctl = E.ctl;
  const int G = (int)gridDim.x;
  const bool timer = E.ktime != nullptr && blockIdx.x == 0 && threadIdx.x == 0;
  unsigned long long tk = timer ? gcn_wall_clock() : 0ull;
#define KT_LAP(SLOT) do { if (timer) { const unsigned long long now_ = gcn_wall_clock(); s_ktime[SLOT] += now_ - tk; tk = now_; } } while (0)
  if (E.ktime) { for (int k = threadIdx.x; k < KT_N; k += BS) s_ktime[k] = 0ull; __syncthreads(); }
#define KT_FLUSH() do { if (E.ktime) { __syncthreads(); for (int k_ = threadIdx.x; k_ < KT_N; k_ += BS) if (k_ != KT_SUB_LAST && k_ != KT_SUB_LAST + 1) { const unsigned long long v_ = s_ktime[k_]; if (v_) { atomicAdd(&E.ktime[k_], v_); s_ktime[k_] = 0ull; } } } } while (0)
  if (ctl->state != 0) {
    if (blockIdx.x == 0 && threadIdx.x == 0) *E.hexit = ordinal;
    return;
  }
  if (ordinal == E.fail_ordinal) {
    if (blockIdx.x == 0 && threadIdx.x == 0) tail_fail(E, TAIL_FAIL_ENTRY);
    return;
  }
  uint32_t epoch = E.psync->gen;
  XBar xb{E.xbar && G > 1 ? 1 : 0, 0u};
  if (xb.on && threadIdx.x == 0) { L.xcc = gcn_xcc_id(); gcn_add_agent(&E.psync->xcount[L.xcc][0], 1u); }
  if (!grid_sync<BS>(E, L, epoch, G, [&](auto &&) {
        if (xb.on && threadIdx.x < 8) {
          PSync *ps = E.psync;
          const uint32_t n = gcn_load_agent(&ps->xcount[threadIdx.x][0]);
          gcn_store_agent(&ps->xn[threadIdx.x][0], n);
          gcn_store_agent(&ps->xcount[threadIdx.x][0], 0u);
          gcn_store_agent(&ps->xarr[threadIdx.x][0], 0u);
          gcn_store_agent(&ps->xgen[threadIdx.x][0], 0u);
          L.xtmp[threadIdx.x] = (int)n;
        }
        if (xb.on) {
          __syncthreads();
          if (threadIdx.x == 0) {
            uint32_t ng = 0;
            for (int g = 0; g < 8; g++) ng += L.xtmp[g] != 0;
            gcn_store_agent(&E.psync->ngrp, ng);
            gcn_store_agent(&E.psync->top, 0u);
          }
        }
        if (threadIdx.x == 0) {
          const int seq = ctl->pub_seq + 1;
          int ex = 0;
          if (seq - ctl->hcons_seen > E.ring_limit) {
            const int hc = gcn_load_system((const int32_t *)E.hcons);
            ctl->hcons_seen = hc;
            if (seq - hc > E.ring_limit) ex = 1;
          }
          if (ctl->pf_wait) {
            const uint32_t seq = (uint32_t)ctl->pf_wait;
            uint32_t done = gcn_load_agent(&E.pfsync->done);
            const unsigned long long t0 = gcn_wall_clock();
            while ((int32_t)(done - seq) < 0 && gcn_wall_clock() - t0 < E.pf_wait_ticks) { gcn_poll_pause(); done = gcn_load_agent(&E.pfsync->done); }
            if ((int32_t)(done - seq) < 0) ex = 1; else ctl->pf_wait = 0;
          }
          ctl->kexit = ex;
          ctl->need_compare = 0;
          if (ex) {
            if (ctl->nalign > 0) ctl->nalign_ran = ctl->nalign;
            ctl->nbatch = 0; ctl->nalign = 0;
          }
        }
      }, TAIL_FAIL_ENTRY))
    return;
  if (ctl->kexit) {
    if (blockIdx.x == 0 && threadIdx.x == 0) *E.hexit = ordinal;
    return;
  }
  if (xb.on) {
    if (threadIdx.x == 0) { L.xn = (int)gcn_load_agent(&E.psync->xn[L.xcc][0]); L.ngrp = (int)gcn_load_agent(&E.psync->ngrp); }
    __syncthreads();
  }
  if (mir) mir_fill<BS>(E, mir);
  KT_LAP(KT_LAUNCH);
  for (int rnd = 0;; rnd++) {
    const int ring = ctl->pub_seq % RING2;
    Round2Out *out = E.dblk + ring;
    int level = 0;
    const bool shuffles = !(first && rnd == 0);
    if (shuffles) {
      shuffle_body<true, BS>(E, L.sh, 0, 0, E.movers, out, nullptr, BudKey{1.0, 0u}, nullptr, mir);
      KT_LAP(KT_S0);
      if (!grid_sync<BS>(E, L, epoch, G, [](auto &&) {}, TAIL_FAIL_LATE, &xb)) return;
      KT_LAP(KT_S0_BAR);
      level = 1;
    }
    int moved = shuffles ? out->cnt[0] : 0;
    for (;;) {
      const bool more = shuffles && level < E.max_shuffle && out->cnt[level - 1] > 0;
      int32_t *mv = E.movers + (size_t)level * 3 * (size_t)E.S.N;
      const bool attempt = more && E.spec_eval && out->cnt[level - 1] <= E.spec_max_prev;
      if (more && !attempt) {
        shuffle_body<false, BS>(E, L.sh, level, moved, mv, out, nullptr, BudKey{1.0, 0u}, nullptr, mir);
        KT_LAP(KT_SL);
        if (!grid_sync<BS>(E, L, epoch, G, [](auto &&) {}, TAIL_FAIL_LATE, &xb)) return;
        KT_LAP(KT_SL_BAR);
        moved += out->cnt[level];
        level++;
        continue;
      }
      if (more) { shuffle_body<false, BS, true>(E, L.sh, level, moved, mv, out, &L.pu, init, (BudKey *)E.partial, mir); KT_LAP(KT_SL); }
      else { pupdate_body<BS>(E, L.pu, level, init, (BudKey *)E.partial, mir); KT_LAP(KT_P); }
      const int lv = level;
      if (!grid_sync<BS>(E, L, epoch, G, [&](auto &&release) {
            if (more && out->cnt[lv] != 0) {
              if (threadIdx.x == 0) *E.sig_n = 0;
              return;
            }
            const int nlev = more ? lv + 1 : lv;
            const unsigned long long tb = E.ktime ? gcn_wall_clock() : 0ull;
            static_assert(sizeof(ShufLds<BS>) - offsetof(ShufLds<BS>, s_work) >= sizeof(uint32_t) * KB_MAX * NKMER && offsetof(ShufLds<BS>, s_work) % 16 == 0, "ShufLds lends 32 KB to birth_body");
            birth_body<true>(E, nlev, Chain2{nlev, true}, init, (const BudKey *)E.partial, G, ordinal, [&]() {
              if (threadIdx.x == 0) {
                ctl->pub_seq = ctl->pub_seq + 1;
                if (E.ktime) { atomicAdd(&E.ktime[KT_BIRTH], gcn_wall_clock() - tb); atomicAdd(&E.ktime[KT_ROUNDS], 1ull); atomicAdd(&E.ktime[KT_LEVELS], (unsigned long long)nlev); }
              }
              release();
            }, (uint32_t *)L.sh.s_work);
          }, TAIL_FAIL_LATE, &xb))
        return;
      if (!more) { KT_LAP(KT_P_BAR); break; }
      KT_LAP(KT_SL_BAR);
      moved += out->cnt[level];
      level++;
      if (out->cnt[level - 1] == 0) {
        if (E.greedy) spec_locks_flush<BS>(E, L.pu, out, mir);
        break;
      }
    }
    const bool leave = ctl->kexit != 0;
    if (mir && out->birth_applied) {
      const int raw = ctl->centre;
      if (threadIdx.x == 0 && (raw >> 6) % G == (int)blockIdx.x) mir_set(mir, raw, MIR_CL | MIR_LOCK, (uint32_t)(ctl->nclust - 1) & MIR_CL);
    }
    if (E.mirror_on == 2) mir_verify<BS>(E, mir);
    KT_FLUSH();
    if (L.last) {
      const unsigned long long tp = E.ktime ? gcn_wall_clock() : 0ull;
      publish_copy(E, out, ring, ctl->pub_seq);
      if (threadIdx.x == 0) {
        if (leave) *E.hexit = ordinal;
        if (E.ktime) atomicAdd(&E.ktime[KT_PUBLISH], gcn_wall_clock() - tp);
      }
    }
    if (leave) return;
  }
#undef KT_LAP
#undef KT_FLUSH
}

constexpr int TAIL_BS = 1024;
struct TailDev {
  std::once_flag once;
  int ncu = 64;
  int cap = -1;
  bool mirror = false;
};
static TailDev &tail_dev(int device) {
  static TailDev devs[64];
  TailDev &d = devs[device & 63];
  std::call_once(d.once, [&]() {
    int cur = 0;
    const bool have_cur = hipGetDevice(&cur) == hipSuccess;
    if (have_cur && cur != device) (void)hipSetDevice(device);
    hipDeviceProp_t prop;
    const bool have_prop = hipGetDeviceProperties(&prop, device) == hipSuccess && prop.multiProcessorCount > 0;
    if (have_prop) d.ncu = prop.multiProcessorCount;
    const void *fn = (const void *)k3_tail<TAIL_BS>;
    const size_t lds_m = tail_lds_bytes<TAIL_BS>(true), lds_0 = tail_lds_bytes<TAIL_BS>(false);
    size_t lds = lds_m;
    bool settable = true;
    d.mirror = hipFuncSetAttribute(fn, hipFuncAttributeMaxDynamicSharedMemorySize, (int)lds_m) == hipSuccess;
    if (d.mirror) {
      int per_cu = 0;
      if (hipOccupancyMaxActiveBlocksPerMultiprocessor(&per_cu, fn, TAIL_BS, lds_m) == hipSuccess && per_cu <= 0) d.mirror = false;
    }
    if (!d.mirror) {
      (void)hipGetLastError();
      lds = lds_0;
      settable = hipFuncSetAttribute(fn, hipFuncAttributeMaxDynamicSharedMemorySize, (int)lds_0) == hipSuccess;
    }
    int per_cu = 0;
    if (!settable) { (void)hipGetLastError(); d.cap = 0; }
    else if (hipOccupancyMaxActiveBlocksPerMultiprocessor(&per_cu, fn, TAIL_BS, lds) != hipSuccess || !have_prop) { (void)hipGetLastError(); d.cap = -1; }
    else d.cap = std::max(0, per_cu) * d.ncu;
    if (have_cur && cur != device) (void)hipSetDevice(cur);
  });
  return d;
}
int tail_resident_max(int device) { return tail_dev(device).cap; }
int tail_mirror_cap(int device) { return tail_dev(device).mirror ? MIR_CAP : 0; }
int tail_grid(int N, int device) {
  const int want = (N + 4095) / 4096;
  return std::max(1, std::min(want, tail_dev(device).ncu));
}
void launch3_tail(const Eng2 &E, int grid, bool first, int ordinal, uint32_t init_reads, hipStream_t st) {
  BudKey init{1.0, init_reads};
  int dev_ = 0;
  (void)hipGetDevice(&dev_);
  (void)tail_dev(dev_);
  hipLaunchKernelGGL(k3_tail<TAIL_BS>, dim3(grid), dim3(TAIL_BS), tail_lds_bytes<TAIL_BS>(E.mirror_on != 0), st, E, init, first ? 1 : 0, ordinal);
}
```

### include/dada2hip.h

```cpp
#ifndef DADA2HIP_H
#define DADA2HIP_H

#include <stddef.h>
#include <stdint.h>

#ifdef __cplusplus
extern "C" {
#endif

#define DADA2HIP_OK            0
#define DADA2HIP_ERR_INPUT     1
#define DADA2HIP_ERR_DEVICE    2
#define DADA2HIP_ERR_RUNTIME   3
#define DADA2HIP_ERR_UNSUPPORTED 4
#define DADA2HIP_ERR_ABORTED   5
#define DADA2HIP_ERR_INTERNAL  6

#define DADA2HIP_NA_INTEGER (-2147483647 - 1)

typedef struct dada2hip_opts {
  double kdist_cutoff, omegaA, omegaP, omegaC, min_fold;
  int32_t match, mismatch, gap, homo_gap, band_size, max_clust, min_hamming, min_abund;
  int32_t use_kmers, detect_singletons, use_quals, final_consensus, vectorized_alignment;
  int32_t multithread, verbose, SSE, gapless, greedy;
} dada2hip_opts;

typedef struct dada2hip_hooks {
  void (*log)(const char *msg, void *user);
  int (*should_abort)(void *user);
  void *user;
} dada2hip_hooks;

typedef struct dada2hip_sample dada2hip_sample;
typedef struct dada2hip_result dada2hip_result;

typedef struct dada2hip_stats {
  uint64_t ncompare;
  uint64_t nskipped;
  uint64_t nshroud;
  uint64_t ngapless;
  uint64_t nnw;
  uint64_t nshuffle;
  uint64_t nstored;
  uint32_t rounds;
  uint32_t kernel_times_sampled;
  double ms_total, ms_upload, ms_screen, ms_nw, ms_gapless, ms_bookkeep, ms_pval, ms_final;
  double nw_kernel_ms;
  uint64_t nw_kernel_launches;
  uint64_t nw_cells;
  double screen_kernel_ms;
  uint64_t screen_kernel_launches;
  uint64_t screen_bytes;
  double dev_ms_screen, dev_ms_nw, dev_ms_shuffle, dev_ms_pval, dev_ms_birth, dev_ms_final;
  double ms_wait_device, ms_replay, ms_enqueue;
  uint64_t nmoves, batch_compares;
  uint64_t nnw_run, ngapless_run;
  uint64_t lite_chains, lite_misses;
  uint64_t tail_launches, tail_pauses, tail_levels;
  uint32_t tail_blocks;
  uint32_t tail_fallbacks;
  double dev_ms_tail, tail_ms_entry, tail_ms_shuffle0, tail_ms_shuffle_more, tail_ms_pupdate, tail_ms_barriers, tail_ms_birth,
      tail_ms_publish, tail_ms_release;
  uint64_t pf_compares, pf_hits, pf_waits, pf_exits, pf_centres;
  uint32_t tail_threads, overlap_on;
  double dev_ms_pf_screen, dev_ms_pf_nw;
  uint32_t tail_xcd_barrier;
  uint32_t tail_mirror;
  double ms_setup, ms_round0;
  double tail_ms_pf_wait, tail_ms_pf_plan;
  uint64_t nnw_retry, nnw_fast;
  uint64_t screen_stage2;
  uint64_t nnw_rounds;
} dada2hip_stats;

int dada2hip_dada_uniques(int32_t nraw, const char *const *seqs, const int32_t *abundances,
                          const uint8_t *priors, const double *err, int32_t err_ncol, const double *quals,
                          int32_t quals_nrow, const dada2hip_opts *opts, int32_t device,
                          const dada2hip_hooks *hooks, dada2hip_result **out, char *errbuf, size_t errlen);

typedef struct dada2hip_sample_input {
  int32_t nraw;
  int32_t quals_nrow;
  const char *const *seqs;
  const int32_t *abundances;
  const uint8_t *priors;
  const double *quals;
} dada2hip_sample_input;
int dada2hip_run_multi(int32_t n_samples, const dada2hip_sample_input *samples, const double *err, int32_t err_ncol,
                       const dada2hip_opts *opts, int32_t n_devices, const int32_t *device_ids, dada2hip_result **out,
                       char *errbuf, size_t errlen);

void dada2hip_trim_cache(void);

int dada2hip_sample_create(int32_t nraw, const char *const *seqs, const int32_t *abundances,
                           const uint8_t *priors, const double *quals, int32_t quals_nrow, int32_t device,
                           dada2hip_sample **out, char *errbuf, size_t errlen);
int dada2hip_sample_set_priors(dada2hip_sample *s, const uint8_t *priors, char *errbuf, size_t errlen);
#define DADA2HIP_PRIOR_SEQS_NSTATS 16
int dada2hip_sample_set_prior_seqs(dada2hip_sample *s, int32_t n, const char *const *seqs, const uint8_t *or_flags,
                                   int32_t *first_match, int32_t *nset, char *errbuf, size_t errlen);
void dada2hip_sample_prior_seqs_stats(const dada2hip_sample *s, int64_t *stats);
int dada2hip_sample_run(dada2hip_sample *s, const double *err, int32_t err_ncol, const dada2hip_opts *opts,
                        const dada2hip_hooks *hooks, dada2hip_result **out, char *errbuf, size_t errlen);
void dada2hip_sample_free(dada2hip_sample *s);

typedef struct dada2hip_shard {
  int32_t rank, world;
  int (*exchange)(void *user, int32_t kind, const void *send, int64_t send_bytes, void *recv);
  void *user;
} dada2hip_shard;
int dada2hip_sample_run_sharded(dada2hip_sample *s, const double *err, int32_t err_ncol, const dada2hip_opts *opts,
                                const dada2hip_hooks *hooks, const dada2hip_shard *shard, dada2hip_result **out,
                                char *errbuf, size_t errlen);
int32_t dada2hip_sample_nraw(const dada2hip_sample *s);
int32_t dada2hip_sample_maxlen(const dada2hip_sample *s);

int32_t dada2hip_result_nclust(const dada2hip_result *r);
int32_t dada2hip_result_nraw(const dada2hip_result *r);
int32_t dada2hip_result_maxlen(const dada2hip_result *r);
int32_t dada2hip_result_ncol(const dada2hip_result *r);
int32_t dada2hip_result_nbirth_subs(const dada2hip_result *r);
const char *dada2hip_result_sequence(const dada2hip_result *r, int32_t i);
const int32_t *dada2hip_result_abundance(const dada2hip_result *r);
const int32_t *dada2hip_result_n0(const dada2hip_result *r);
const int32_t *dada2hip_result_n1(const dada2hip_result *r);
const int32_t *dada2hip_result_nunq(const dada2hip_result *r);
const double *dada2hip_result_clust_pval(const dada2hip_result *r);
const int32_t *dada2hip_result_birth_from(const dada2hip_result *r);
const double *dada2hip_result_birth_pval(const dada2hip_result *r);
const double *dada2hip_result_birth_fold(const dada2hip_result *r);
const int32_t *dada2hip_result_birth_ham(const dada2hip_result *r);
const double *dada2hip_result_birth_qave(const dada2hip_result *r);
const int32_t *dada2hip_result_center(const dada2hip_result *r);
const int32_t *dada2hip_result_bs_pos(const dada2hip_result *r);
const char *dada2hip_result_bs_ref(const dada2hip_result *r);
const char *dada2hip_result_bs_sub(const dada2hip_result *r);
const double *dada2hip_result_bs_qual(const dada2hip_result *r);
const int32_t *dada2hip_result_bs_clust(const dada2hip_result *r);
const int32_t *dada2hip_result_subqual(const dada2hip_result *r);
const double *dada2hip_result_clusterquals(const dada2hip_result *r);
const int32_t *dada2hip_result_map(const dada2hip_result *r);
const double *dada2hip_result_pval(const dada2hip_result *r);
void dada2hip_result_stats(const dada2hip_result *r, dada2hip_stats *out);
void dada2hip_result_free(dada2hip_result *r);

int dada2hip_nwalign(const char *s1, const char *s2, int32_t match, int32_t mismatch, int32_t gap_p,
                     int32_t homo_gap_p, int32_t band, int32_t endsfree, int32_t device, char *out0, char *out1,
                     char *errbuf, size_t errlen);
int dada2hip_nwvec(int32_t n, const char *const *s1, const char *const *s2, int32_t match, int32_t mismatch,
                   int32_t gap_p, int32_t band, int32_t endsfree, int32_t device, char *const *out,
                   char *errbuf, size_t errlen);

int dada2hip_table_bimera2(int32_t nrow, int32_t ncol, const int32_t *mat, const char *const *seqs, double min_fold,
                           int32_t min_abund, int32_t allow_one_off, int32_t min_one_off_par_dist, int32_t match,
                           int32_t mismatch, int32_t gap_p, int32_t max_shift, int32_t device, int32_t *nflag, int32_t *nsam,
                           char *errbuf, size_t errlen);
int dada2hip_is_bimera(const char *sq, int32_t npars, const char *const *pars, int32_t allow_one_off,
                       int32_t min_one_off_par_dist, int32_t match, int32_t mismatch, int32_t gap_p, int32_t max_shift,
                       int32_t device, int32_t *out, char *errbuf, size_t errlen);
int dada2hip_bimera_pairs(int32_t n, const char *const *queries, const char *const *parents, int32_t allow_one_off,
                          int32_t match, int32_t mismatch, int32_t gap_p, int32_t max_shift, int32_t device, int32_t *out,
                          char *errbuf, size_t errlen);

#define DADA2HIP_BIMERA_DENOVO_NSTATS 16
int dada2hip_bimera_denovo(int32_t nrow, int32_t ncol, const int32_t *mat, const char *const *seqs, double min_fold,
                           double min_parent_abund, int32_t allow_one_off, int32_t min_one_off_par_dist, int32_t match,
                           int32_t mismatch, int32_t gap_p, int32_t max_shift, int32_t skip_zero, int32_t device, uint8_t *flags,
                           int64_t *stats, char *errbuf, size_t errlen);

int dada2hip_bimera_worklist_probe(int32_t n, const int32_t *rank, const int32_t *P, const uint8_t *flags, int32_t nq,
                                   const int32_t *live, int32_t r0, int32_t wr, int32_t per, int32_t device, int32_t *chunk_centre,
                                   int32_t *work, char *errbuf, size_t errlen);
int dada2hip_bimera_fold_probe(int32_t n, const int32_t *len, const int32_t *P, int32_t nq, const int32_t *live, int32_t r0,
                               int32_t wr, const int32_t *work, const int32_t *rec, int32_t allow_one_off,
                               int32_t min_one_off_par_dist, int32_t last, int32_t device, int32_t *maxima, uint8_t *flags,
                               int32_t *next_live, int32_t *n_next, int64_t *aligned, char *errbuf, size_t errlen);

typedef struct dada2hip_derep dada2hip_derep;
int dada2hip_derep_fastq(const char *path, int64_t chunk_reads, int32_t qual_offset, dada2hip_derep **out, char *errbuf,
                         size_t errlen);
int32_t dada2hip_derep_nuniques(const dada2hip_derep *d);
int64_t dada2hip_derep_nreads(const dada2hip_derep *d);
int32_t dada2hip_derep_maxlen(const dada2hip_derep *d);
const char *const *dada2hip_derep_seqs(const dada2hip_derep *d);
const int32_t *dada2hip_derep_abundances(const dada2hip_derep *d);
const double *dada2hip_derep_quals(const dada2hip_derep *d);
const int32_t *dada2hip_derep_map(const dada2hip_derep *d);
void dada2hip_derep_free(dada2hip_derep *d);
int dada2hip_sample_from_derep(const dada2hip_derep *d, const uint8_t *priors, int32_t device, dada2hip_sample **out,
                               char *errbuf, size_t errlen);

#define DADA2HIP_DEREP_NSTATS 16
int dada2hip_derep_reads(int64_t n, const char *seq, const char *qual, const int64_t *offsets, int64_t chunk_reads,
                         int32_t qual_offset, int32_t device, dada2hip_derep **out, int64_t *stats, char *errbuf, size_t errlen);

typedef struct dada2hip_derep_view {
  int32_t nuniques, maxlen;
  int64_t nreads;
  const char *const *seqs;
  const int32_t *abundances;
  const double *quals;
  const int32_t *map;
} dada2hip_derep_view;
int dada2hip_derep_combine(int32_t nsamples, const dada2hip_derep_view *in, dada2hip_derep **out, int32_t *unique_to_pool,
                           char *errbuf, size_t errlen);

typedef struct dada2hip_mergers dada2hip_mergers;
int dada2hip_merge_pairs(int64_t nreads, const int32_t *fwd, const int32_t *rev, int32_t nF, const char *const *seqsF,
                         const int32_t *n0F, int32_t nR, const char *const *seqsR, const int32_t *n0R, int32_t min_overlap,
                         int32_t max_mismatch, int32_t trim_overhang, int32_t just_concatenate, int32_t device,
                         dada2hip_mergers **out, char *errbuf, size_t errlen);
int32_t dada2hip_mergers_nrow(const dada2hip_mergers *m);
const char *dada2hip_mergers_sequence(const dada2hip_mergers *m, int32_t i);
const int32_t *dada2hip_mergers_abundance(const dada2hip_mergers *m);
const int32_t *dada2hip_mergers_forward(const dada2hip_mergers *m);
const int32_t *dada2hip_mergers_reverse(const dada2hip_mergers *m);
const int32_t *dada2hip_mergers_nmatch(const dada2hip_mergers *m);
const int32_t *dada2hip_mergers_nmismatch(const dada2hip_mergers *m);
const int32_t *dada2hip_mergers_nindel(const dada2hip_mergers *m);
const int32_t *dada2hip_mergers_prefer(const dada2hip_mergers *m);
const int32_t *dada2hip_mergers_accept(const dada2hip_mergers *m);
void dada2hip_mergers_free(dada2hip_mergers *m);

#define DADA2HIP_COLLAPSE_NSTATS 16
int dada2hip_collapse_nomismatch(int32_t nrow, int32_t ncol, const int32_t *mat, const char *const *seqs, int32_t min_overlap,
// ... 160 lines not shown
```

Before: 7.823 million.

## Have the persistent tail report exit reasons and enqueue compare chains only when due

The persistent round-tail kernel now writes an exit reason record (why it stopped, whether a compare is due, prefetch state, halt code, sequence) into host-visible flags. The host reads this to decide whether the next relaunch needs the screen/NW compare chain, rather than always attaching it, and holds off speculative relaunches when the device is paused or halted. A cmp_seq marker set after each compare chain makes resume and entry logic check that the compare actually ran for the current round. This is meant to cut redundant screen/alignment launches and wasted tail launches, at the cost of extra host polling logic and new sequencing invariants.

```diff
diff --git a/dada2_amd/_lib.py b/dada2_amd/_lib.py
--- a/dada2_amd/_lib.py
+++ b/dada2_amd/_lib.py
@@ -44,10 +44,13 @@
         ("tail_xcd_barrier", C.c_uint32), ("tail_mirror", C.c_uint32),
         ("ms_setup", C.c_double), ("ms_round0", C.c_double), ("tail_ms_pf_wait", C.c_double), ("tail_ms_pf_plan", C.c_double),
         ("nnw_retry", C.c_uint64), ("nnw_fast", C.c_uint64), ("screen_stage2", C.c_uint64), ("nnw_rounds", C.c_uint64),
+        ("tail_exit_reason", C.c_uint64 * 8),
+        ("compare_chains_sent", C.c_uint64), ("compare_chains_needed", C.c_uint64), ("tail_mover_halts", C.c_uint64),
     ]
 
     def as_dict(self):
-        return {k: getattr(self, k) for k, _ in self._fields_ if not k.startswith("reserved")}
+        d = {k: getattr(self, k) for k, _ in self._fields_ if not k.startswith("reserved")}
+        return {k: list(v) if isinstance(v, C.Array) else v for k, v in d.items()}
 
 
 EXCHANGE_FN = C.CFUNCTYPE(C.c_int, C.c_void_p, C.c_int32, C.c_void_p, C.c_int64, C.c_void_p)
diff --git a/dada2_amd/csrc/driver.cpp b/dada2_amd/csrc/driver.cpp
--- a/dada2_amd/csrc/driver.cpp
+++ b/dada2_amd/csrc/driver.cpp
@@ -1416,7 +1416,8 @@
     E2.sp = sp; E2.thresh = d_thresh_round.p; E2.max_shuffle = MAX_SHUFFLE;
     E2.trace = v2_trace.p; E2.trace_seq = v2_trace_seq;
     E2.moved = v2_moved.p; E2.n0d = v2_n0d.p; E2.stat_part = v2_statpart.p; E2.stat_n = v2_n0d.p + 2 * SH_LEVELS;
-    E2.psync = v3_psync.p; E2.hcons = v3_hflags.p; E2.hexit = v3_hflags.p ? v3_hflags.p + 16 : nullptr; E2.ktime = v3_ktime.p;
+    E2.psync = v3_psync.p; E2.hcons = v3_hflags.p; E2.hexit = v3_hflags.p ? v3_hflags.p + 16 : nullptr;
+    E2.hreason = v3_hflags.p ? v3_hflags.p + 48 : nullptr; E2.ktime = v3_ktime.p;
     E2.sh_filter = 1; E2.grid_shuffle = 2048; E2.grid_pupdate = 1024;
     const Knobs &K = knobs();
     if (K.v2_filter >= 0) E2.sh_filter = K.v2_filter;
@@ -1622,11 +1623,49 @@
   bool v3_block_ready() const { return *(volatile int32_t *)&v2_hblk.p[v2_cons % RING2].seq == (int32_t)(v2_cons + 1); }
   long v3_ended() const { return (long)*(volatile int32_t *)(v3_hflags.p + 16); }
   std::vector<EnqRec> v3_rec;
-  void v3_enqueue(bool first) {
+  long v3_reason_ord = 0;
+  long v3_answered = 0;
+  uint64_t v3_nreason[8] = {0, 0, 0, 0, 0, 0, 0, 0}, v3_chains_sent = 0, v3_chains_needed = 0;
+  bool v3_informed() const { return v3_depth == 1 && !knobs().v3_blind; }
+  bool v3_reason_valid() const { return v3_enq > 0 && v3_ended() == v3_enq; }
+  int32_t v3_reason(int k) const { return *(volatile int32_t *)(v3_hflags.p + 48 + k); }
+  void v3_reason_count() {
+    if (!v3_reason_valid() || v3_reason_ord == v3_enq) return;
+    std::atomic_thread_fence(std::memory_order_acquire);
+    v3_reason_ord = v3_enq;
+    v3_nreason[v3_reason(0) & 7]++;
+  }
+  bool v3_hold() {
+    if (!v3_informed() || !v3_reason_valid()) return false;
+    v3_reason_count();
+    const int why = v3_reason(0);
+    if (why == TX_HALTED_BEFORE && v3_reason(3) == H2_FAIL) return true;
+    if (why == TX_PF_NOT_READY && v3_overlap) {
+      const long pw = (long)v3_reason(2);
+      const bool running = pw > 0 && pw <= v3_pf_launched && v3_pf_gate_result(pw) != 2;
+      if (!running && (long)v3_reason(4) > v2_cons) return true;
+    }
+    return (why ==TX_PAUSE || why == TX_HALT_HOST || why == TX_HALT_END || why == TX_HALTED_BEFORE) && (long)v3_reason(4) > v3_answered;
+  }
+  void v3_enqueue(bool first, int chain = -1) {
     const auto t_enq = clk::now();
     hipStream_t stq = s->stream;
-    EnqRec rec{-1, -1, !first};
-    if (!first) {
+    bool with_chain = !first;
+    v3_reason_count();
+    if (!first && v3_informed() && (chain >= 0 || v3_reason_valid())) {
+      if (chain >= 0) with_chain = chain != 0;
+      else {
+        v3_reason_count();
+        with_chain = v3_reason(1) != 0;
+        const long pw = (long)v3_reason(2);
+        if (v3_overlap && pw > 0 && pw <= v3_pf_launched) D2_HIP(hipStreamWaitEvent(stq, v3_pf_ev[pw & 3], 0));
+      }
+      if (with_chain && chain != 2) v3_chains_needed++;
+      if (with_chain && knobs().v3_skip_compare > 0 && v3_enq + 1 == (long)knobs().v3_skip_compare) with_chain = false;
+    }
+    EnqRec rec{-1, -1, with_chain};
+    if (with_chain) {
+      v3_chains_sent++;
       rec.ev_screen = ev_begin(EV_SCREEN, profile_all, true);
       launch2_screen_multi(E2, stq);
       ev_end(rec.ev_screen);
@@ -1637,6 +1676,7 @@
       launch_nw_ad(s->D, -1, nullptr, nullptr, nullptr, 0, nullptr, nullptr, ap, s->d_err.p, v2_lamB.p, v2_hamB.p, nullptr, 0, 0, nullptr, stq,
                    &v2_ctl.p->state, &nb);
       ev_end(rec.ev_nw);
+      launch2_cmp_done(E2, stq);
     }
     const int ev = ev_begin(EV_TAIL, profile_all);
     Eng2 Ek = E2;
@@ -1699,7 +1739,7 @@
   bool v3_dev_halted = false;
 
   void v3_topup() {
-    if (v3_dev_halted) return;
+    if (v3_dev_halted || v3_hold()) return;
     const long need = (long)v3_depth - (v3_enq - v3_ended());
     for (long k = 0; k < need; k++) v3_enqueue(false);
   }
@@ -1711,7 +1751,7 @@
     const bool polite = wait_blocks();
     int burst = 0;
     for (unsigned spins = 0; *seqp != want; spins++) {
-      if (v3_enq - v3_ended() < v3_depth && burst < 256) { v3_enqueue(false); burst++; continue; }
+      if (v3_enq - v3_ended() < v3_depth && burst < 256 && !v3_hold()) { v3_enqueue(false); burst++; continue; }
       cpu_relax();
       if (polite && spins > 64) { struct timespec ts{0, 20000}; nanosleep(&ts, nullptr); }
       if ((spins & 0xFFFF) == 0xFFFF || (polite && (spins & 0xFF) == 0xFF)) {
@@ -1719,7 +1759,7 @@
         if (e != hipSuccess && e != hipErrorNotReady)
           throw d2::DeviceError{DADA2HIP_ERR_DEVICE, std::string("HIP error: ") + hipGetErrorString(e) + " (round result)"};
         if (e == hipSuccess && *seqp != want) {
-          if (v3_ended() < v3_enq || burst >= 2) {
+          if (v3_ended() < v3_enq || burst >= 2 || v3_hold()) {
             PSync ps;
             D2_HIP(hipMemcpy(&ps, v3_psync.p, sizeof ps, hipMemcpyDeviceToHost));
             if (ps.fail == 1u) throw TailEntryFailed{};
@@ -1745,16 +1785,20 @@
     st.nstored = (uint64_t)N;
     v3_rec.clear();
     if (v3_overlap && v3_pf_gate_on && (active_runs(s->device).load() <= 1 || knobs().v3_overlap == 1)) v3_pf_enqueue(1);
+    v3_reason_ord = 0; v3_answered = 0; v3_chains_sent = v3_chains_needed = 0;
+    for (auto &n : v3_nreason) n = 0;
     v3_enqueue(true);
+    if (v3_informed()) v3_enqueue(false, 2);
     bool done = false;
     long n_halt[8] = {0, 0, 0, 0, 0, 0, 0, 0}, n_pause = 0, n_blocks = 0;
     while (!done) {
-      for (int burst = 0; !v3_dev_halted && v3_enq - v3_ended() < v3_depth && burst < 4; burst++) v3_enqueue(false);
+      for (int burst = 0; !v3_dev_halted && v3_enq - v3_ended() < v3_depth && burst < 4 && !v3_hold(); burst++) v3_enqueue(false);
       const long seq = v2_cons + 1;
       const Round2Out *bp = nullptr;
       try { bp = &v3_wait_block(); }
       catch (const TailEntryFailed &) {
         v3_running = false;
+        st.tail_exit_reason[TX_ENTRY_FAILED]++;
         v3_fallback();
         st.ms_bookkeep += ms_since(t0);
         run_v2(max_clust, true, v2_cons == 0);
@@ -1773,8 +1817,10 @@
       v2_replay(b, seq, b.paused != 0 && b.halt == H2_NONE);
       n_halt[b.halt & 7]++;
       if (b.kord > v3_ord_seen) {
+        EnqRec rec{-1, -1, false};
+        for (long q = b.kord; q > v3_ord_seen; q--)
+          if (v3_rec[(size_t)q - 1].compare) { rec = v3_rec[(size_t)q - 1]; break; }
         v3_ord_seen = b.kord;
-        const EnqRec &rec = v3_rec[(size_t)b.kord - 1];
         if (rec.compare && b.pad0[1] + b.pad0[2] > 0) {
           if (rec.ev_nw >= 0) evs[rec.ev_nw].ok = 1;
           st.nnw_run += (uint64_t)b.pad0[1]; st.ngapless_run += (uint64_t)b.pad0[2];
@@ -1820,6 +1866,7 @@
         default: throw RuntimeErr{DADA2HIP_ERR_RUNTIME, "dada2hip: internal error: unexpected halt code from the persistent round tail"};
       }
       v3_dev_halted = false;
+      v3_answered = std::max(v3_answered, seq);
       *(volatile int32_t *)v3_hflags.p = (int32_t)v2_cons;
     }
     v3_running = false;
@@ -1847,6 +1894,15 @@
     }
     st.tail_xcd_barrier = (E2.xbar && v3_grid > 1) ? 1u : 0u;
     st.tail_mirror = (v3_enq > 0 && E2.mirror_on) ? 1u : 0u;
+    v3_reason_count();
+    for (int k = 0; k < 8; k++) st.tail_exit_reason[k] = v3_nreason[k];
+    st.compare_chains_sent = v3_chains_sent; st.compare_chains_needed = v3_chains_needed;
+    st.tail_mover_halts = (uint64_t)n_pause;
+    if (knobs().v2_summary)
+      fprintf(stderr, "[v3] exits compare/prefetch/ring/pause/halt-host/halt-end/halted-before/entry %llu %llu %llu %llu %llu %llu %llu %llu  compare chains sent %llu needed %llu  mover halts %ld\n",
+              (unsigned long long)v3_nreason[0], (unsigned long long)v3_nreason[1], (unsigned long long)v3_nreason[2], (unsigned long long)v3_nreason[3],
+              (unsigned long long)v3_nreason[4], (unsigned long long)v3_nreason[5], (unsigned long long)v3_nreason[6], (unsigned long long)v3_nreason[7],
+              (unsigned long long)v3_chains_sent, (unsigned long long)v3_chains_needed, n_pause);
     st.tail_launches = (uint64_t)v3_enq; st.tail_pauses = (uint64_t)n_pause; st.tail_blocks = (uint32_t)v3_grid; st.tail_threads = 1024;
     if (knobs().v2_summary && v3_overlap)
       fprintf(stderr, "[v3] overlap: prefetch compares %ld in %ld chains (centres %d)  rounds served from a prefetched batch %d  waits inside the launch %d  launches left for one %d\n",
@@ -1945,7 +2001,8 @@
       D2_HIP(hipStreamSynchronize(s->side));
       if (resume_after_fetch) {
         launch2_resume(E2, s->stream, true);
-        v3_enqueue(false);
+        v3_answered = std::max(v3_answered, seq);
+        v3_enqueue(false, v3_informed() ? (b.next_compare != 0 ? 1 : 0) : -1);
       }
       off = 0;
       for (int l = 0; l < b.nsh; l++) { replay_moves(h_big.p + 3 * off, b.cnt[l]); off += (size_t)b.cnt[l]; }
diff --git a/dada2_amd/csrc/engine.h b/dada2_amd/csrc/engine.h
--- a/dada2_amd/csrc/engine.h
+++ b/dada2_amd/csrc/engine.h
@@ -264,6 +264,10 @@
 };
 
 enum : int32_t { H2_NONE = 0, H2_NO_BIRTH, H2_HOST_DECIDE, H2_SHUFFLE_MORE, H2_CAPACITY, H2_MAXCLUST, H2_NEED_COMPARE, H2_FAIL };
+
+enum : int32_t { TX_COMPARE_DUE = 0, TX_PF_NOT_READY, TX_RING_FULL, TX_PAUSE, TX_HALT_HOST ,
+                 TX_HALT_END , TX_HALTED_BEFORE ,
+                 TX_ENTRY_FAILED , TX_N };
 
 struct Ctl2 {
   int32_t state;
@@ -291,7 +295,8 @@
   int32_t prev_bbuf;
   int32_t pf_hits, pf_spins, pf_exits, pf_centres;
   unsigned long long pf_mask;
-  int32_t fast_off, fast_off_pad;
+  int32_t fast_off;
+  int32_t cmp_seq;
 };
 
 struct Cache2 {
@@ -322,7 +327,8 @@
   int32_t pf_seq;
   int32_t pf_wait;
   int32_t pf_stat[4];
-  int32_t pad1[2];
+  int32_t next_compare;
+  int32_t pad1;
   int32_t kord;
   int32_t paused;
   unsigned long long stat[4];
@@ -370,6 +376,7 @@
   struct PSync *psync;
   volatile int32_t *hcons;
   volatile int32_t *hexit;
+  volatile int32_t *hreason;
   unsigned long long *ktime;
   int32_t xbar;
   int32_t spec_max_prev;
@@ -413,6 +420,7 @@
 void launch2_pf_gate(const Eng2 &E, int k, const int32_t *h_quit, int32_t *h_result, hipStream_t st);
 void launch2_pf_tables(const Eng2 &E, hipStream_t st);
 void launch2_pf_done(const Eng2 &E, hipStream_t st);
+void launch2_cmp_done(const Eng2 &E, hipStream_t st);
 void launch2_batch_lists(const Eng2 &E, hipStream_t st);
 void launch2_shuffle(const Eng2 &E, int level, bool store, hipStream_t st);
 void launch2_eval(const Eng2 &E, int nlev, uint32_t init_reads, hipStream_t st);
diff --git a/dada2_amd/csrc/knobs.h b/dada2_amd/csrc/knobs.h
--- a/dada2_amd/csrc/knobs.h
+++ b/dada2_amd/csrc/knobs.h
@@ -41,6 +41,8 @@
   int v3_slots = 3;
   int v3_mirror = 1;
   int v3_fail_entry = 0;
+  int v3_skip_compare = 0;
+  int v3_blind = 0;
   bool v2_debug = false;
   bool v2_summary = false;
   bool v2_trace_on = false;
@@ -111,7 +113,8 @@
     if (const char *e = S("DADA2HIP_V2_TAIL")) k.v2_tail_chain = !std::strcmp(e, "chain");
     k.v3_grid = I("DADA2HIP_V3_GRID", 0); k.v3_ring = I("DADA2HIP_V3_RING", 0);
     k.v3_overlap = T("DADA2HIP_V3_OVERLAP"); k.v3_pf_wait_us = I("DADA2HIP_V3_PF_WAIT_US", -1);
-    k.v3_fail_entry = I("DADA2HIP_V3_FAIL_ENTRY", 0); k.v3_spec = I("DADA2HIP_V3_SPEC", 1); k.v3_xbar = T("DADA2HIP_V3_XBAR"); k.v3_spec_max = I("DADA2HIP_V3_SPEC_MAX", -1);
+    k.v3_fail_entry = I("DADA2HIP_V3_FAIL_ENTRY", 0); k.v3_skip_compare = I("DADA2HIP_V3_SKIP_COMPARE", 0); k.v3_blind = I("DADA2HIP_V3_BLIND", 0);
+    k.v3_spec = I("DADA2HIP_V3_SPEC", 1); k.v3_xbar = T("DADA2HIP_V3_XBAR"); k.v3_spec_max = I("DADA2HIP_V3_SPEC_MAX", -1);
     k.v3_pf_early = I("DADA2HIP_V3_PF_EARLY", -1); k.v3_pf_sync = I("DADA2HIP_V3_PF_SYNC", 0); k.v3_pf_gate_us = I("DADA2HIP_V3_PF_GATE_US", -1);
     k.v3_mirror = I("DADA2HIP_V3_MIRROR", 1);
     k.v3_slots = I("DADA2HIP_V3_SLOTS", 3);
diff --git a/dada2_amd/csrc/rounds2.inc.hip b/dada2_amd/csrc/rounds2.inc.hip
--- a/dada2_amd/csrc/rounds2.inc.hip
+++ b/dada2_amd/csrc/rounds2.inc.hip
@@ -1345,13 +1345,20 @@
     if (pause) { out->paused = 1; ctl->state = 1; ctl->halt = H2_NONE; }
     out->kord = kord;
     const int seq = ctl->pub_seq + 1;
-    int ex = (s_halt != H2_NONE || pause || ctl->need_compare != 0 || E.align_at_commit != 0 || ctl->pf_wait != 0) ? 1 : 0;
+    const int cmp_due = (s_halt == H2_NONE && (ctl->need_compare != 0 || E.align_at_commit != 0)) ? 1 : 0;
+    int ex = (s_halt != H2_NONE || pause || cmp_due || ctl->pf_wait != 0) ? 1 : 0;
+    int why = s_halt != H2_NONE ? ((s_halt == H2_NO_BIRTH || s_halt == H2_MAXCLUST) ? TX_HALT_END : TX_HALT_HOST)
+              : pause ? TX_PAUSE : cmp_due ? TX_COMPARE_DUE : TX_PF_NOT_READY;
     if (!ex && seq + 1 - s_pre[PRE_HCONS] > E.ring_limit) {
       const int hc = gcn_load_system((const int32_t *)E.hcons);
       ctl->hcons_seen = hc;
-      if (seq + 1 - hc > E.ring_limit) ex = 1;
+      if (seq + 1 - hc > E.ring_limit) { ex = 1; why = TX_RING_FULL; }
     }
     ctl->kexit = ex;
+    out->next_compare = cmp_due;
+    if (ex && E.hreason) {
+      E.hreason[0] = why; E.hreason[1] = cmp_due; E.hreason[2] = ctl->pf_wait; E.hreason[3] = s_halt; E.hreason[4] = seq;
+    }
   }
   clear_block(E.dblk + ((ring + 1) % RING2));
   go();
@@ -1404,7 +1411,7 @@
 __global__ void k2_resume(Eng2 E, int keep_list, int compare_done) {
   E.ctl->state = 0; E.ctl->halt = H2_NONE;
   if (!keep_list) *E.sig_n = 0;
-  if (compare_done) { E.ctl->nbatch = 0; E.ctl->need_compare = 0; if (!E.align_at_commit) E.ctl->nalign = 0; }
+  if (compare_done && E.ctl->cmp_seq == E.ctl->pub_seq + 1) { E.ctl->nbatch = 0; E.ctl->need_compare = 0; if (!E.align_at_commit) E.ctl->nalign = 0; }
 }
 
 __global__ void k2_pf_gate(Eng2 E, int k, const int32_t *quit, int32_t *result) {
@@ -1426,6 +1433,10 @@
   const int nb = E.ctl->nbatch;
   if (E.ctl->state != 0 || nb <= 0) return;
   build_batch_tables(E.S, E.C, nb, E.ctl->bcentre, s_cnt);
+}
+__global__ void k2_cmp_done(Eng2 E) {
+  if (threadIdx.x != 0 || E.ctl->state != 0) return;
+  E.ctl->cmp_seq = E.ctl->pub_seq + 1;
 }
 __global__ void k2_pf_done(Eng2 E) {
   if (threadIdx.x != 0 || E.ctl->state != 0) return;
@@ -1699,6 +1710,7 @@
 }
 void launch2_pf_tables(const Eng2 &E, hipStream_t st) { hipLaunchKernelGGL(k2_pf_tables, dim3(1), dim3(1024), 0, st, E); }
 void launch2_pf_done(const Eng2 &E, hipStream_t st) { hipLaunchKernelGGL(k2_pf_done, dim3(1), dim3(64), 0, st, E); }
+void launch2_cmp_done(const Eng2 &E, hipStream_t st) { hipLaunchKernelGGL(k2_cmp_done, dim3(1), dim3(64), 0, st, E); }
 void launch2_screen_multi(const Eng2 &E, hipStream_t st) {
   const size_t lds = (size_t)NKMER * 8 + (size_t)KB_MAX * E.S.LK * 2 + (size_t)(E.S.maxlen + 2) * 4 + 16;
   static size_t attr_set[64] = {0};
diff --git a/dada2_amd/csrc/rounds3.inc.hip b/dada2_amd/csrc/rounds3.inc.hip
--- a/dada2_amd/csrc/rounds3.inc.hip
+++ b/dada2_amd/csrc/rounds3.inc.hip
@@ -14,6 +14,14 @@
 static __device__ __forceinline__ void tail_fail(const Eng2 &E, uint32_t code) {
   gcn_store_agent(&E.psync->fail, code);
   E.ctl->state = 1; E.ctl->halt = H2_FAIL;
+}
+
+static __device__ __forceinline__ void tail_exit(const Eng2 &E, int ordinal, int why, int cmp_due, int pf_wait, int halt, int seq) {
+  if (E.hreason) {
+    E.hreason[0] = why; E.hreason[1] = cmp_due; E.hreason[2] = pf_wait; E.hreason[3] = halt; E.hreason[4] = seq;
+    __threadfence_system();
+  }
+  *E.hexit = ordinal;
 }
 
 template <int BS, typename F>
@@ -153,7 +161,7 @@
   if (E.ktime) { for (int k = threadIdx.x; k < KT_N; k += BS) s_ktime[k] = 0ull; __syncthreads(); }
 #define KT_FLUSH() do { if (E.ktime) { __syncthreads(); for (int k_ = threadIdx.x; k_ < KT_N; k_ += BS) if (k_ != KT_SUB_LAST && k_ != KT_SUB_LAST + 1) { const unsigned long long v_ = s_ktime[k_]; if (v_) { atomicAdd(&E.ktime[k_], v_); s_ktime[k_] = 0ull; } } } } while (0)
   if (ctl->state != 0) {
-    if (blockIdx.x == 0 && threadIdx.x == 0) *E.hexit = ordinal;
+    if (blockIdx.x == 0 && threadIdx.x == 0) tail_exit(E, ordinal, TX_HALTED_BEFORE, 0, 0, ctl->halt, ctl->pub_seq);
     return;
   }
   if (ordinal == E.fail_ordinal) {
@@ -184,7 +192,14 @@
         }
         if (threadIdx.x == 0) {
           const int seq = ctl->pub_seq + 1;
-          int ex = 0;
+          int ex = 0, why = TX_RING_FULL;
+          const bool due = !first && (ctl->need_compare != 0 || (E.align_at_commit != 0 && ctl->nalign > 0));
+          const bool unran = due && ctl->cmp_seq != seq;
+          if (unran) {
+            ctl->kexit = 1;
+            tail_exit(E, ordinal, TX_COMPARE_DUE, 1, ctl->pf_wait, H2_NONE, seq - 1);
+            return;
+          }
           if (seq - ctl->hcons_seen > E.ring_limit) {
             const int hc = gcn_load_system((const int32_t *)E.hcons);
             ctl->hcons_seen = hc;
@@ -195,21 +210,19 @@
             uint32_t done = gcn_load_agent(&E.pfsync->done);
             const unsigned long long t0 = gcn_wall_clock();
             while ((int32_t)(done - seq) < 0 && gcn_wall_clock() - t0 < E.pf_wait_ticks) { gcn_poll_pause(); done = gcn_load_agent(&E.pfsync->done); }
-            if ((int32_t)(done - seq) < 0) ex = 1; else ctl->pf_wait = 0;
+            if ((int32_t)(done - seq) < 0) { ex = 1; why = TX_PF_NOT_READY; } else ctl->pf_wait = 0;
           }
           ctl->kexit = ex;
           ctl->need_compare = 0;
           if (ex) {
             if (ctl->nalign > 0) ctl->nalign_ran = ctl->nalign;
             ctl->nbatch = 0; ctl->nalign = 0;
+            tail_exit(E, ordinal, why, 0, ctl->pf_wait, H2_NONE, seq - 1);
           }
         }
       }, TAIL_FAIL_ENTRY))
     return;
-  if (ctl->kexit) {
-    if (blockIdx.x == 0 && threadIdx.x == 0) *E.hexit = ordinal;
-    return;
-  }
+  if (ctl->kexit) return;
   if (xb.on) {
     if (threadIdx.x == 0) { L.xn = (int)gcn_load_agent(&E.psync->xn[L.xcc][0]); L.ngrp = (int)gcn_load_agent(&E.psync->ngrp); }
     __syncthreads();
diff --git a/include/dada2hip.h b/include/dada2hip.h
--- a/include/dada2hip.h
+++ b/include/dada2hip.h
@@ -71,6 +71,8 @@
   uint64_t nnw_retry, nnw_fast;
   uint64_t screen_stage2;
   uint64_t nnw_rounds;
+  uint64_t tail_exit_reason[8];
+  uint64_t compare_chains_sent, compare_chains_needed, tail_mover_halts;
 } dada2hip_stats;
 
 int dada2hip_dada_uniques(int32_t nraw, const char *const *seqs, const int32_t *abundances,
```

Measured after the change: 7.641 million. 2.3% lower.
